# xUhEngwAng/I2V-Adapter-Unofficial

Hardware: AMD Instinct MI355X
Metric: denoising steps/sec @ 16fx512x512 SD1.5+I2V-Adapter (higher is better)
Workload: dtype f16

## Files before the change

### i2v-adapter-unofficial_amd/_lib.py

```python
import ctypes as C
import os

_HERE = os.path.dirname(os.path.abspath(__file__))
LIB_PATH = os.environ.get("I2V_LIB_PATH") or os.path.join(_HERE, "libi2v_hip.so")
ABI_VERSION = 27

I2V_EPI_NONE, I2V_EPI_GELU, I2V_EPI_GEGLU = 0, 1, 2
I2V_STORE_ROWMAJOR, I2V_STORE_ROWPERM, I2V_STORE_VT, I2V_STORE_VT_T = 0, 1, 2, 3
I2V_A_PLAIN, I2V_A_CONV3X3 = 0, 1
I2V_LORA_MAX_ADAPTERS, I2V_LORA_MAX_RANK = 8, 256
I2V_ROUTE_GENERIC, I2V_ROUTE_CONV_THIN, I2V_ROUTE_BIG_TILE, I2V_ROUTE_BIG_DEEP, I2V_ROUTE_BIG_SPLITK = 0, 1, 2, 3, 4
I2V_EXTRA_NONE, I2V_EXTRA_LNF, I2V_EXTRA_HILO, I2V_EXTRA_GNS, I2V_EXTRA_UPF = 0, 1, 2, 4, 8
I2V_TATTN_LDS_FORM, I2V_TATTN_REG_FORM = 0, 1
I2V_ADD_RES_MAX = 16
I2V_TAESD_PREP_IDENTITY, I2V_TAESD_PREP_UNIT, I2V_TAESD_PREP_CLAMP = 0, 1, 2


class HipLibraryError(RuntimeError):
    pass


class GemmParams(C.Structure):
    _fields_ = [
        ("a", C.c_void_p), ("lda", C.c_int64),
        ("a2", C.c_void_p), ("lda2", C.c_int64),
        ("k_split", C.c_int32), ("a_mode", C.c_int32),
        ("w", C.c_void_p), ("ldw", C.c_int64),
        ("bias", C.c_void_p),
        ("residual", C.c_void_p), ("ldr", C.c_int64),
        ("rowvec", C.c_void_p), ("ld_rowvec", C.c_int64), ("rows_per_vec", C.c_int32), ("rowvec_period", C.c_int32),
        ("ln_wsum", C.c_void_p), ("ln_eps", C.c_float),
        ("c", C.c_void_p), ("ldc", C.c_int64),
        ("M", C.c_int32), ("N", C.c_int32), ("K", C.c_int32),
        ("epilogue", C.c_int32), ("store_mode", C.c_int32),
        ("frames", C.c_int32), ("hw", C.c_int32),
        ("vt_len", C.c_int32), ("vt_ld", C.c_int32),
        ("out_scale", C.c_float),
        ("n_img", C.c_int32), ("in_h", C.c_int32), ("in_w", C.c_int32), ("cin", C.c_int32),
        ("out_h", C.c_int32), ("out_w", C.c_int32), ("stride", C.c_int32), ("upsample", C.c_int32),
        ("asym_pad", C.c_int32), ("conv_kblock", C.c_int32),
        ("w_batch_stride", C.c_int64), ("rows_per_w", C.c_int32),
        ("a_perm_frames", C.c_int32), ("a_perm_hw", C.c_int32),
        ("workspace", C.c_void_p), ("workspace_bytes", C.c_int64),
        ("c_is_f32", C.c_int32),
        ("gn_partial", C.c_void_p), ("gn_groups", C.c_int32),
        ("residual_lo", C.c_void_p), ("c_lo", C.c_void_p),
    ]


class GemmRoute(C.Structure):
    _fields_ = [
        ("family", C.c_int32), ("a_mode", C.c_int32),
        ("rows", C.c_int32), ("cols", C.c_int32), ("stages", C.c_int32),
        ("splits", C.c_int32), ("kps", C.c_int32),
        ("extra", C.c_int32), ("persistent", C.c_int32),
        ("generic_tile", C.c_int32), ("vec4", C.c_int32),
        ("epilogue", C.c_int32), ("store_mode", C.c_int32),
    ]

    def as_dict(self):
        return {name: int(getattr(self, name)) for name, _ in self._fields_}


class AttnParams(C.Structure):
    _fields_ = [
        ("q", C.c_void_p), ("q_row_stride", C.c_int64), ("q_batch_stride", C.c_int64),
        ("k", C.c_void_p), ("k_row_stride", C.c_int64), ("k_batch_stride", C.c_int64),
        ("vt", C.c_void_p), ("vt_row_stride", C.c_int64), ("vt_batch_stride", C.c_int64),
        ("o", C.c_void_p), ("o_row_stride", C.c_int64), ("o_batch_stride", C.c_int64),
        ("batch_q", C.c_int32), ("kv_group", C.c_int32), ("heads", C.c_int32), ("head_dim", C.c_int32),
        ("lq", C.c_int32), ("lk", C.c_int32),
        ("scale", C.c_float), ("accumulate", C.c_int32), ("acc_scale", C.c_float),
        ("lse", C.c_void_p),
    ]


class AttnBwdParams(C.Structure):
    _fields_ = [
        ("q", C.c_void_p), ("q_row_stride", C.c_int64), ("q_batch_stride", C.c_int64),
        ("qt", C.c_void_p), ("qt_row_stride", C.c_int64), ("qt_batch_stride", C.c_int64),
        ("k", C.c_void_p), ("k_row_stride", C.c_int64), ("k_batch_stride", C.c_int64),
        ("kt", C.c_void_p), ("kt_row_stride", C.c_int64), ("kt_batch_stride", C.c_int64),
        ("v", C.c_void_p), ("v_row_stride", C.c_int64), ("v_batch_stride", C.c_int64),
        ("dout", C.c_void_p), ("do_row_stride", C.c_int64), ("do_batch_stride", C.c_int64),
        ("doutt", C.c_void_p), ("dot_row_stride", C.c_int64), ("dot_batch_stride", C.c_int64),
        ("lse", C.c_void_p), ("delta", C.c_void_p),
        ("dq", C.c_void_p), ("dq_row_stride", C.c_int64), ("dq_batch_stride", C.c_int64),
        ("dk", C.c_void_p), ("dk_row_stride", C.c_int64), ("dk_batch_stride", C.c_int64),
        ("dv", C.c_void_p), ("dv_row_stride", C.c_int64), ("dv_batch_stride", C.c_int64),
        ("batch_q", C.c_int32), ("kv_group", C.c_int32), ("heads", C.c_int32), ("head_dim", C.c_int32),
        ("lq", C.c_int32), ("lk", C.c_int32),
        ("scale", C.c_float), ("kv_partitions", C.c_int32), ("dkv_partial", C.c_void_p),
    ]


class TAttnParams(C.Structure):
    _fields_ = [
        ("q", C.c_void_p), ("q_row_stride", C.c_int64),
        ("k", C.c_void_p), ("k_row_stride", C.c_int64),
        ("vt", C.c_void_p), ("vt_ld", C.c_int32),
        ("o", C.c_void_p), ("o_row_stride", C.c_int64),
        ("n_pixels", C.c_int32), ("frames", C.c_int32), ("heads", C.c_int32), ("head_dim", C.c_int32),
        ("scale", C.c_float),
    ]


class TAttnRoute(C.Structure):
    _fields_ = [
        ("form", C.c_int32), ("dqk", C.c_int32), ("dpv", C.c_int32),
        ("pf", C.c_int32), ("nqt", C.c_int32), ("blocks", C.c_int32),
    ]

    def as_dict(self):
        return {name: int(getattr(self, name)) for name, _ in self._fields_}


class MotionAttnParams(C.Structure):
    _fields_ = [
        ("x", C.c_void_p), ("ldx", C.c_int64),
        ("gamma", C.c_void_p),
        ("shift", C.c_void_p), ("ld_shift", C.c_int64),
        ("w_qkv", C.c_void_p),
        ("out", C.c_void_p), ("ldo", C.c_int64),
        ("rows", C.c_int64),
        ("channels", C.c_int32), ("heads", C.c_int32), ("head_dim", C.c_int32), ("frames", C.c_int32),
        ("eps", C.c_float), ("scale", C.c_float),
        ("w_o", C.c_void_p), ("b_o", C.c_void_p),
    ]


class CrossAttnFusedParams(C.Structure):
    _fields_ = [
        ("x", C.c_void_p), ("ldx", C.c_int64),
        ("gamma", C.c_void_p), ("beta", C.c_void_p),
        ("w_q", C.c_void_p),
        ("ctx_frag", C.c_void_p),
        ("out", C.c_void_p), ("ldo", C.c_int64),
        ("rows", C.c_int64), ("rows_per_ctx", C.c_int64),
        ("channels", C.c_int32), ("heads", C.c_int32), ("head_dim", C.c_int32), ("ctx_len", C.c_int32),
        ("eps", C.c_float), ("scale", C.c_float),
        ("ip_frag", C.c_void_p), ("ip_len", C.c_int32), ("ip_scale", C.c_float),
        ("w_o", C.c_void_p), ("b_o", C.c_void_p),
    ]


class FfFusedParams(C.Structure):
    _fields_ = [
        ("x", C.c_void_p), ("ldx", C.c_int64),
        ("gamma", C.c_void_p), ("beta", C.c_void_p),
        ("w1", C.c_void_p), ("b1", C.c_void_p),
        ("w2", C.c_void_p), ("b2", C.c_void_p),
        ("out", C.c_void_p), ("ldo", C.c_int64),
        ("rows", C.c_int64),
        ("channels", C.c_int32), ("inner", C.c_int32),
        ("eps", C.c_float),
        ("w3", C.c_void_p), ("b3", C.c_void_p),
        ("res2", C.c_void_p), ("ld_res2", C.c_int64),
        ("perm_frames", C.c_int32), ("perm_hw", C.c_int32),
        ("res2_lo", C.c_void_p), ("out_lo", C.c_void_p),
    ]


class LnQkvParams(C.Structure):
    _fields_ = [
        ("x", C.c_void_p), ("ldx", C.c_int64),
        ("gamma", C.c_void_p), ("beta", C.c_void_p),
        ("w", C.c_void_p),
        ("qk", C.c_void_p), ("ld_qk", C.c_int64),
        ("vt", C.c_void_p), ("vt_batch_stride", C.c_int64), ("vt_row_stride", C.c_int64),
        ("rows", C.c_int64), ("rows_per_image", C.c_int64),
        ("channels", C.c_int32), ("n_qk", C.c_int32),
        ("eps", C.c_float),
        ("x_image_stride", C.c_int64),
    ]


class UnetConfig(C.Structure):
    _fields_ = [
        ("in_channels", C.c_int32), ("out_channels", C.c_int32),
        ("block_out_channels", C.c_int32 * 4),
        ("layers_per_block", C.c_int32), ("num_attention_heads", C.c_int32),
        ("cross_attention_dim", C.c_int32), ("norm_num_groups", C.c_int32),
        ("motion_max_seq_length", C.c_int32), ("motion_num_attention_heads", C.c_int32),
        ("use_motion_mid_block", C.c_int32), ("ip_num_tokens", C.c_int32),
    ]


class UnetPlan(C.Structure):
    _fields_ = [
        ("batch", C.c_int32), ("frames", C.c_int32), ("height", C.c_int32), ("width", C.c_int32),
        ("ctx_len", C.c_int32), ("has_ip", C.c_int32),
    ]


class GnParams(C.Structure):
    _fields_ = [
        ("x", C.c_void_p), ("c1", C.c_int32),
        ("x2", C.c_void_p), ("c2", C.c_int32),
        ("gamma", C.c_void_p), ("beta", C.c_void_p),
        ("y", C.c_void_p),
        ("n_img", C.c_int32), ("hw", C.c_int32), ("groups", C.c_int32), ("frames_per_stat", C.c_int32),
        ("eps", C.c_float), ("silu", C.c_int32),
        ("out_perm", C.c_int32), ("frames", C.c_int32),
        ("workspace", C.c_void_p),
        ("gpartial_in", C.c_void_p), ("gpartial_rows", C.c_int32),
    ]


class LoraAdapter(C.Structure):
    _fields_ = [("down", C.c_void_p), ("up", C.c_void_p), ("rank", C.c_int32), ("scale", C.c_float)]


class LnParams(C.Structure):
    _fields_ = [
        ("x", C.c_void_p), ("ldx", C.c_int64),
        ("gamma", C.c_void_p), ("beta", C.c_void_p),
        ("pe", C.c_void_p), ("ld_pe", C.c_int64), ("pe_period", C.c_int32),
        ("y", C.c_void_p), ("ldy", C.c_int64),
        ("rows", C.c_int32), ("C", C.c_int32),
        ("eps", C.c_float),
        ("x_rows_per_batch", C.c_int32), ("x_batch_stride", C.c_int64),
    ]


class AddResidualsEntry(C.Structure):
    _fields_ = [("dst", C.c_void_p), ("dst_lo", C.c_void_p), ("skip", C.c_void_p), ("skip_lo", C.c_void_p), ("res", C.c_void_p),
                ("numel", C.c_int64)]


class AddResidualsParams(C.Structure):
    _fields_ = [("t", AddResidualsEntry * I2V_ADD_RES_MAX), ("n", C.c_int32), ("scale_rows", C.c_int32), ("scale_table", C.c_void_p),
                ("step_idx", C.c_void_p)]


class ConvC64Params(C.Structure):
    _fields_ = [
        ("x", C.c_void_p), ("ldx", C.c_int64),
        ("w", C.c_void_p), ("bias", C.c_void_p),
        ("residual", C.c_void_p), ("ldr", C.c_int64),
        ("out", C.c_void_p), ("ldo", C.c_int64),
        ("n_img", C.c_int32), ("height", C.c_int32), ("width", C.c_int32),
        ("cin", C.c_int32), ("cout", C.c_int32),
        ("relu_mid", C.c_int32), ("relu_out", C.c_int32),
        ("max_workgroups", C.c_int32),
    ]


_P = C.c_void_p
SIGNATURES = {
    "i2v_abi_version": (C.c_int, []),
    "i2v_last_error": (C.c_char_p, []),
    "i2v_gemm_f16": (C.c_int, [C.POINTER(GemmParams), _P]),
    "i2v_gemm_ln_supported": (C.c_int, [C.POINTER(GemmParams)]),
    "i2v_gemm_batch_supported": (C.c_int, [C.POINTER(GemmParams)]),
    "i2v_gemm_upconv_fold_supported": (C.c_int, [C.POINTER(GemmParams)]),
    "i2v_gemm_workspace_bytes": (C.c_int64, [C.POINTER(GemmParams)]),
    "i2v_gemm_gn_partial_rows": (C.c_int32, [C.POINTER(GemmParams)]),
    "i2v_gemm_route": (C.c_int, [C.POINTER(GemmParams), C.POINTER(GemmRoute)]),
    "i2v_gemm_last_route": (C.c_int, [C.POINTER(GemmRoute)]),
    "i2v_gemm_kernel_exists": (C.c_int, [C.POINTER(GemmRoute)]),
    "i2v_attention_f16": (C.c_int, [C.POINTER(AttnParams), _P]),
    "i2v_temporal_attention_f16": (C.c_int, [C.POINTER(TAttnParams), _P]),
    "i2v_temporal_attention_route": (C.c_int, [C.POINTER(TAttnParams), C.POINTER(TAttnRoute)]),
    "i2v_temporal_attention_last_route": (C.c_int, [C.POINTER(TAttnRoute)]),
    "i2v_tattn_kernel_exists": (C.c_int, [C.POINTER(TAttnRoute)]),
    "i2v_motion_attn_supported": (C.c_int32, [C.c_int64, C.c_int32, C.c_int32, C.c_int32, C.c_int32]),
    "i2v_motion_attn_pack_rows": (C.c_int32, [C.c_int32, C.c_int32]),
    "i2v_motion_attn_f16": (C.c_int, [C.POINTER(MotionAttnParams), _P]),
    "i2v_cross_attn_fused_supported": (C.c_int32, [C.c_int64, C.c_int32, C.c_int32, C.c_int32, C.c_int32, C.c_int64]),
    "i2v_cross_attn_fused_pack_rows": (C.c_int32, [C.c_int32, C.c_int32]),
    "i2v_cross_attn_fused_ctx_elems": (C.c_int64, [C.c_int32, C.c_int32, C.c_int32]),
    "i2v_cross_attn_fused_f16": (C.c_int, [C.POINTER(CrossAttnFusedParams), _P]),
    "i2v_ln_qkv_supported": (C.c_int32, [C.c_int64, C.c_int32, C.c_int32, C.c_int64]),
    "i2v_ln_qkv_f16": (C.c_int, [C.POINTER(LnQkvParams), _P]),
    "i2v_ff_fused_supported": (C.c_int32, [C.c_int64, C.c_int32, C.c_int32]),
    "i2v_ff_fused_tail_supported": (C.c_int32, [C.c_int64, C.c_int32, C.c_int32, C.c_int32, C.c_int32]),
    "i2v_ff_fused_f16": (C.c_int, [C.POINTER(FfFusedParams), _P]),
    "i2v_groupnorm_workspace_bytes": (C.c_int64, [C.c_int32, C.c_int32, C.c_int32]),
    "i2v_groupnorm_f16": (C.c_int, [C.POINTER(GnParams), _P]),
    "i2v_groupnorm_fold_f16": (C.c_int, [C.POINTER(GnParams), _P, C.c_int64, _P, C.c_int32, _P, _P, _P]),
    "i2v_layernorm_f16": (C.c_int, [C.POINTER(LnParams), _P]),
    "i2v_softmax_rows_f16": (C.c_int, [_P, C.c_int64, _P, C.c_int64, C.c_int32, C.c_int32, C.c_float, _P]),
    "i2v_nchw_to_tokens": (C.c_int, [_P, C.c_int32, _P, C.c_int32, C.c_int32, C.c_int32, C.c_int32, _P]),
    "i2v_tokens_to_nchw": (C.c_int, [_P, C.c_int32, C.c_int64, _P, C.c_int32, C.c_int32, C.c_int32, C.c_int32, _P]),
    "i2v_timestep_embedding": (C.c_int, [_P, _P, C.c_int32, _P, C.c_int32, C.c_int32, _P]),
    "i2v_silu_f16": (C.c_int, [_P, _P, C.c_int64, _P]),
    "i2v_repeat_rows_f16": (C.c_int, [_P, _P, C.c_int64, C.c_int64, C.c_int32, _P]),
    "i2v_copy3d_f16": (C.c_int, [_P, C.c_int64, C.c_int64, _P, C.c_int64, C.c_int64, C.c_int64, C.c_int64,
                                 C.c_int64, _P]),
    "i2v_pack_ctx_fragments_elems": (C.c_int64, [C.c_int32, C.c_int32, C.c_int32]),
    "i2v_pack_ctx_fragments_f16": (C.c_int, [_P, C.c_int64, _P, C.c_int64, C.c_int64, _P, C.c_int32, C.c_int32, C.c_int32, C.c_int32, _P]),
    "i2v_ddim_prep": (C.c_int, [_P, _P, _P, C.c_int32, C.c_int32, C.c_int32, C.c_int32, C.c_int32, C.c_int32, _P]),
    "i2v_gaussian_sample_f32": (C.c_int, [_P, _P, _P, C.c_int32, C.c_int32, C.c_int32, _P]),
    "i2v_first_frame_prior_f32": (C.c_int, [_P, _P, _P, _P, C.c_int32, C.c_int32, C.c_int32, C.c_int32, C.c_int32,
                                            C.c_float, C.c_float, C.c_float, C.c_float, C.c_float, _P]),
    "i2v_attention_lse_f32": (C.c_int, [C.POINTER(AttnParams), _P, _P]),
    "i2v_attention_bwd_f16": (C.c_int, [C.POINTER(AttnBwdParams), _P]),
    "i2v_transpose_f16": (C.c_int, [_P, C.c_int64, C.c_int64, _P, C.c_int64, C.c_int64, C.c_int32, C.c_int32, C.c_int32, _P]),
    "i2v_rowdot_heads_f32": (C.c_int, [_P, C.c_int64, _P, C.c_int64, _P, C.c_int64, C.c_int32, C.c_int32, C.c_int32, _P]),
    "i2v_layernorm_bwd_f16": (C.c_int, [_P, C.c_int64, _P, C.c_int64, _P, _P, C.c_int64, _P, C.c_int64, C.c_int32, C.c_int32,
                                        C.c_float, _P]),
    "i2v_geglu_bwd_f16": (C.c_int, [_P, C.c_int64, _P, C.c_int64, _P, C.c_int64, C.c_int64, C.c_int32, _P]),
    "i2v_geglu_f16": (C.c_int, [_P, C.c_int64, _P, C.c_int64, C.c_int64, C.c_int32, _P]),
    "i2v_colsum_f32": (C.c_int, [_P, C.c_int64, _P, C.c_int64, C.c_int32, _P]),
    "i2v_colsum_prod_f32": (C.c_int, [_P, C.c_int64, _P, C.c_int64, _P, C.c_int64, C.c_int32, _P]),
    "i2v_colsum_workspace_bytes": (C.c_int64, [C.c_int64, C.c_int32]),
    "i2v_colsum_det_f32": (C.c_int, [_P, C.c_int64, _P, C.c_int64, _P, C.c_int64, C.c_int32, _P, _P]),
    "i2v_masked_mse_grad_f16": (C.c_int, [_P, _P, _P, C.c_int64, C.c_int32, C.c_int32, C.c_int32, C.c_float, _P]),
    "i2v_masked_mse_grad_f32": (C.c_int, [_P, _P, _P, _P, C.c_int64, C.c_int32, C.c_int32, C.c_int32, C.c_float, _P]),
    "i2v_groupnorm_bwd_workspace_bytes": (C.c_int64, [C.c_int32, C.c_int32, C.c_int32]),
    "i2v_groupnorm_bwd_f16": (C.c_int, [C.POINTER(GnParams), _P, _P, _P, _P]),
    "i2v_add_f16": (C.c_int, [_P, _P, _P, C.c_int64, _P]),
    "i2v_permute_rows_f16": (C.c_int, [_P, _P, C.c_int64, C.c_int32, C.c_int32, C.c_int32, C.c_int32, _P]),
    "i2v_zero_insert2x_f16": (C.c_int, [_P, _P, C.c_int64, C.c_int32, C.c_int32, C.c_int32, _P]),
    "i2v_sum_pool2x_f16": (C.c_int, [_P, _P, C.c_int64, C.c_int32, C.c_int32, C.c_int32, _P]),
    "i2v_sumsq_f32": (C.c_int, [_P, C.c_int64, _P, _P]),
    "i2v_adamw_f32": (C.c_int, [_P, _P, _P, _P, C.c_int64, C.c_float, C.c_float, C.c_float, C.c_float, C.c_float, C.c_int32,
                                C.c_float, _P, C.c_float, _P]),
    "i2v_adamw_guarded_f32": (C.c_int, [_P, _P, _P, _P, C.c_int64, C.c_float, C.c_float, C.c_float, C.c_float, C.c_float,
                                        C.c_float, C.c_float, _P, C.c_int32, _P, _P, _P, _P]),
    "i2v_axpby_f32": (C.c_int, [_P, _P, C.c_float, C.c_float, C.c_int64, _P]),
    "i2v_select_row_f16": (C.c_int, [_P, C.c_int64, C.c_int32, _P, _P, C.c_int32, _P]),
    "i2v_ddim_cfg_step": (C.c_int, [_P, _P, C.c_int32, C.c_int64, _P, C.c_int32, _P, C.c_float, C.c_int32, C.c_int32,
                                    C.c_int32, C.c_int32, C.c_int32, _P]),
    "i2v_dpm_cfg_step": (C.c_int, [_P, _P, _P, C.c_int32, C.c_int64, _P, C.c_int32, _P, C.c_float, C.c_int32, C.c_int32,
                                   C.c_int32, C.c_int32, C.c_int32, _P]),
    "i2v_lcm_cfg_step": (C.c_int, [_P, _P, C.c_int32, _P, C.c_int32, C.c_int64, _P, C.c_int32, _P, C.c_float, C.c_int32, C.c_int32,
                                   C.c_int32, C.c_int32, C.c_int32, _P]),
    "i2v_freeu_f16": (C.c_int, [_P, _P, _P, _P, _P, _P, C.c_int32, C.c_int32, C.c_int32, C.c_int32, C.c_int32, C.c_float, C.c_float, _P]),
    "i2v_vae_tile_blend": (C.c_int, [_P, _P, _P, _P, C.c_int32, C.c_int32, C.c_int32, C.c_int32, C.c_int64, C.c_int32, C.c_int32, C.c_int32,
                                     C.c_int32, C.c_int32, _P, C.c_int32, C.c_int32, C.c_int32, C.c_int32, _P]),
    "i2v_lora_merge": (C.c_int, [_P, _P, C.c_int32, C.c_int32, C.c_int32, C.POINTER(LoraAdapter), C.c_int32, _P]),
    "i2v_freeinit_workspace_bytes": (C.c_int64, [C.c_int32, C.c_int32, C.c_int32, C.c_int32, C.c_int32]),
    "i2v_freeinit_mix": (C.c_int, [_P, _P, _P, _P, _P, _P, C.c_int64, C.c_int32, C.c_int32, C.c_int32, C.c_int32, C.c_int32, C.c_float,
                                   C.c_float, _P]),
    "i2v_freenoise_gather_f16": (C.c_int, [_P, C.c_int64, _P, C.c_int64, _P, C.c_int64, C.c_int32, C.c_int32, C.c_int32, C.c_int32, _P]),
    "i2v_freenoise_blend_f16": (C.c_int, [_P, C.c_int64, _P, C.c_int64, _P, _P, C.c_int64, C.c_int32, C.c_int32, C.c_int32, C.c_int32,
                                          C.c_int32, _P]),
    "i2v_clip_embed_f16": (C.c_int, [_P, _P, _P, _P, _P, C.c_int32, C.c_int32, C.c_int32, C.c_int32, C.c_int32, _P]),
    "i2v_clip_attention_f16": (C.c_int, [_P, C.c_int64, C.c_int32, C.c_int32, C.c_int32, _P, C.c_int64, C.c_int32, C.c_int32, C.c_int32,
                                         C.c_int32, C.c_float, _P]),
    "i2v_quick_gelu_f16": (C.c_int, [_P, _P, C.c_int64, _P]),
    "i2v_clip_patchify_f16": (C.c_int, [_P, _P, C.c_int64, C.c_int32, C.c_int32, C.c_int32, C.c_int32, _P]),
    "i2v_clip_vision_embed_f16": (C.c_int, [_P, _P, C.c_int64, _P, _P, C.c_int32, C.c_int32, C.c_int32, _P]),
    "i2v_clip_vision_attention_f16": (C.c_int, [_P, C.c_int64, C.c_int32, C.c_int32, C.c_int32, _P, C.c_int64, C.c_int32, C.c_int32,
                                                C.c_int32, C.c_int32, C.c_float, _P]),
    "i2v_perceiver_attention_f16": (C.c_int, [_P, C.c_int64, C.c_int32, _P, C.c_int64, C.c_int32, C.c_int32, C.c_int32, _P, C.c_int64,
                                              C.c_int32, C.c_int32, C.c_int32, _P, C.c_int64, C.c_int32, C.c_int32, C.c_int32, C.c_int32,
                                              C.c_float, _P]),
    "i2v_add_residuals_f16": (C.c_int, [C.POINTER(AddResidualsParams), _P]),
    "i2v_conv3x3_c64_f16": (C.c_int, [C.POINTER(ConvC64Params), _P]),
    "i2v_taesd_prep_f16": (C.c_int, [_P, C.c_int32, _P, C.c_int64, C.c_int32, C.c_int32, C.c_int32, C.c_int32, _P]),
    "i2v_pixel_unshuffle8_f16": (C.c_int, [_P, C.c_int32, _P, C.c_int32, C.c_int32, C.c_int32, C.c_int32, _P]),
    "i2v_avgpool2x_f16": (C.c_int, [_P, _P, C.c_int32, C.c_int32, C.c_int32, C.c_int32, _P]),
    "i2v_relu_f16": (C.c_int, [_P, _P, C.c_int64, _P]),
    "i2v_add_broadcast_residual_f16": (C.c_int, [_P, _P, _P, _P, _P, C.c_int64, C.c_int64, _P, C.c_int32, _P, _P]),
    "i2v_interp_rows_f16": (C.c_int, [_P, C.c_int64, C.c_int32, _P, _P, _P, _P, C.c_int64, C.c_int32, C.c_int32, _P]),
    "i2v_masked_renoise_f32": (C.c_int, [_P, _P, _P, _P, _P, C.c_int32, _P, C.c_int64, C.c_int32, C.c_int32, _P]),
    "i2v_weight_embeds_f16": (C.c_int, [_P, _P, _P, _P, C.c_int32, C.c_int32, C.c_int32, C.c_int64, C.c_int64, C.c_int32, _P]),
    "i2v_unet_create": (C.c_int, [C.POINTER(UnetConfig), C.POINTER(_P)]),
    "i2v_unet_destroy": (C.c_int, [_P]),
    "i2v_unet_set_weight": (C.c_int, [_P, C.c_char_p, _P, C.c_int32, C.c_int32, C.POINTER(C.c_int64)]),
    "i2v_unet_get_weight": (C.c_int, [_P, C.c_char_p, C.POINTER(_P), C.POINTER(C.c_int32), C.POINTER(C.c_int32),
                                      C.POINTER(C.c_int64)]),
    "i2v_unet_num_weights": (C.c_int64, [_P]),
    "i2v_unet_plan": (C.c_int, [_P, C.POINTER(UnetPlan)]),
    "i2v_unet_set_plan": (C.c_int, [_P, C.c_char_p, C.c_int64]),
    "i2v_unet_activation_bytes": (C.c_int64, [_P]),
    "i2v_unet_plan_launches": (C.c_int32, [_P]),
    "i2v_unet_plan_num_keys": (C.c_int32, [_P]),
    "i2v_unet_plan_key": (C.c_char_p, [_P, C.c_int32]),
    "i2v_unet_set_workspace": (C.c_int, [_P, _P, C.c_int64]),
    "i2v_unet_forward": (C.c_int, [_P, _P, _P, _P, _P, _P, _P]),
    "i2v_unet_abort_capture": (C.c_int, [_P]),
    "i2v_unet_run": (C.c_int, [_P, C.POINTER(_P), C.c_int32, _P]),
    "i2v_unet_capture_step": (C.c_int, [_P, _P]),
    "i2v_unet_end_capture": (C.c_int, [_P]),
    "i2v_unet_replay_step": (C.c_int, [_P, _P]),
    "i2v_unet_has_step": (C.c_int32, [_P]),
}

_lib = None


def load():
    global _lib
    if _lib is not None:
        return _lib
    if not os.path.exists(LIB_PATH):
        raise HipLibraryError(
            f"{LIB_PATH} not found: the HIP extension is not built.  Run `python __graft_entry__.py build` "
            "(needs hipcc, cross-compiles gfx950 without a GPU).  There is no CPU fallback for this path.")
    try:
        lib = C.CDLL(LIB_PATH)
    except OSError as e:
        raise HipLibraryError(f"cannot load {LIB_PATH}: {e}") from e
    for name, (res, args) in SIGNATURES.items():
        try:
            fn = getattr(lib, name)
        except AttributeError as e:
            raise HipLibraryError(f"{LIB_PATH} does not export `{name}` declared in include/i2v_hip.h") from e
        fn.restype = res
        fn.argtypes = args
    v = lib.i2v_abi_version()
    if v != ABI_VERSION:
        raise HipLibraryError(f"{LIB_PATH} has ABI version {v}, binding expects {ABI_VERSION}")
    _lib = lib
    return lib


def check(status: int, what: str):
    if status != 0:
        msg = load().i2v_last_error()
        raise HipLibraryError(f"{what} failed with status {status}: {msg.decode() if msg else ''}")
```

### i2v-adapter-unofficial_amd/blocks.py

```python
import math
import os
from typing import Optional

import torch
from torch import nn

from . import kernels as K
from . import streams
from ._lib import (I2V_EPI_GEGLU, I2V_EPI_GELU, I2V_EPI_NONE, I2V_STORE_ROWPERM, HipLibraryError)
from .checkpoint import PretrainedMixin

f16 = torch.float16


class HipModule(nn.Module):

    def __init__(self):
        super().__init__()
        self._packed = None
        self._packed_key = None

    def _pack(self):
        return {}

# ... 435 lines not shown
    def refresh_context_fragments(self, pc):
        hit = pc.frag.get(self)
        if hit is not None:
            k, vt, kip, vtip, lt, li = self.context_kv(pc, None)
            K.pack_ctx_fragments(k, vt, self.heads, lt, out=hit[0])
            if hit[1] is not None:
                K.pack_ctx_fragments(kip, vtip, self.heads, li, out=hit[1])

    def _cross(self, q, ctx_text, ctx_ip, batch_q, lq, kv_group, kv=None):
        k, vt, kip, vtip, lt, li = kv if kv is not None else self.context_kv(ctx_text, ctx_ip)
        o = K.attention(q, k, vt, batch_q=batch_q, lq=lq, lk=lt, heads=self.heads, head_dim=self.dim_head,
                        kv_group=kv_group, scale=self.scale)
        if kip is not None and self.ip_num_tokens:
            K.attention(q, kip, vtip, batch_q=batch_q, lq=lq, lk=li, heads=self.heads, head_dim=self.dim_head,
                        kv_group=kv_group, scale=self.scale, out=o, accumulate=True, acc_scale=self.ip_scale)
        return o

    def forward(self, hidden_states, encoder_hidden_states=None, attention_mask=None):
        if attention_mask is not None:
            raise NotImplementedError("attention masks are never passed on the hot path (SURVEY 8b)")
        p = self.packed()
        x = _as_f16_matrix(hidden_states)
        b, l, c = x.shape
        q = K.gemm(x.view(-1, c), p["wq"])
        ctx = x if encoder_hidden_states is None else _as_f16_matrix(encoder_hidden_states)
        ctx_ip = None
        if self.ip_num_tokens and encoder_hidden_states is not None:
            end = ctx.shape[1] - self.ip_num_tokens
            ctx_text = torch.empty((ctx.shape[0], end, ctx.shape[2]), dtype=f16, device=x.device)
            ctx_ip = torch.empty((ctx.shape[0], self.ip_num_tokens, ctx.shape[2]), dtype=f16, device=x.device)
            K.copy3d(ctx[:, :end], ctx_text)
            K.copy3d(ctx[:, end:], ctx_ip)
            ctx = ctx_text
        if b % ctx.shape[0] != 0:
            raise ValueError(f"context batch {ctx.shape[0]} does not divide query batch {b}")
        o = self._cross(q, ctx, ctx_ip, b, l, b // ctx.shape[0])
        out = K.gemm(o, p["wo"], p["bo"])
        return out.view(b, l, -1).to(hidden_states.dtype)


class GEGLU(nn.Module):
    def __init__(self, dim_in, dim_out, bias=True):
        super().__init__()
        self.proj = nn.Linear(dim_in, dim_out * 2, bias=bias)


class GELU(nn.Module):
    def __init__(self, dim_in, dim_out, approximate="none", bias=True):
        super().__init__()
        if approximate != "none":
            raise NotImplementedError("only erf GELU is implemented")
        self.proj = nn.Linear(dim_in, dim_out, bias=bias)


def ff_tail_operands(weight, bias, c_in, c_out):
    if c_in != c_out or not K.ff_fused_tail_supported(128, c_in, 4 * c_in):
        return None
    return K.pack_ff_tail(weight.detach().reshape(c_out, c_in), bias)


class FeedForward(HipModule):

    def __init__(self, dim, dim_out=None, mult=4, dropout=0.0, activation_fn="geglu", inner_dim=None, bias=True):
        super().__init__()
        if not bias:
            raise NotImplementedError("ff_bias=False is not on the hot path")
        inner_dim = int(dim * mult) if inner_dim is None else inner_dim
        dim_out = dim if dim_out is None else dim_out
        self.activation_fn = activation_fn
        if activation_fn == "geglu":
            act = GEGLU(dim, inner_dim, bias=bias)
        elif activation_fn == "gelu":
            act = GELU(dim, inner_dim, bias=bias)
        else:
            raise ValueError(f"unsupported activation_fn {activation_fn}")
        self.net = nn.ModuleList([act, nn.Dropout(dropout), nn.Linear(inner_dim, dim_out, bias=bias)])

    def _pack(self):
        proj = self.net[0].proj
        if self.activation_fn == "geglu":
            w1, b1 = pack_geglu(proj.weight.detach(), proj.bias.detach())
        else:
            w1, b1 = w16(proj.weight), w16(proj.bias)
        out = LazyPack(w1=w1, b1=b1, w2=w16(self.net[2].weight), b2=w16(self.net[2].bias))
        if self.activation_fn == "geglu" and K.ff_fused_supported(128, self.net[2].weight.shape[0], self.net[2].weight.shape[1]):
            out.lazy("fused", lambda proj=proj, lin=self.net[2]: K.pack_ff_fused(proj.weight, proj.bias, lin.weight, lin.bias))
        return out

    def _fwd(self, n2d, residual2d, **store):
        p = self.packed()
        epi = I2V_EPI_GEGLU if self.activation_fn == "geglu" else I2V_EPI_GELU
        h = K.gemm(n2d, p["w1"], p["b1"], epilogue=epi)
        return K.gemm(h, p["w2"], p["b2"], residual=residual2d, **store)

    def fused_supported(self, x2d):
        p = self.packed()
        return FUSED_FF and "fused" in p and K.ff_fused_supported(x2d.shape[0], x2d.shape[1], p["b1"].numel() // 2)

    def _fwd_fused(self, x2d, gamma32, beta32, eps, tail=None):
        return K.ff_fused(x2d, gamma32, beta32, self.packed()["fused"], eps=eps, tail=tail, precise=precise_stream())

    def tail_supported(self, x2d, tail):
        p = self.packed()
        return (FUSED_FF and FUSED_FF_TAIL and tail is not None and tail[0] is not None and "fused" in p and
                K.ff_fused_tail_supported(x2d.shape[0], x2d.shape[1], p["b1"].numel() // 2, tail[2], tail[3]))

    def fold_norm(self, norm):
        if self.activation_fn != "geglu":
            return None
        proj = self.net[0].proj
        return fold_layernorm_geglu(proj.weight, proj.bias, norm.weight, norm.bias)

    def _fwd_folded(self, x2d, eps, folded, **store):
        p = self.packed()
        wf, wsum, bf = folded
        h = K.gemm(x2d, wf, bf, epilogue=I2V_EPI_GEGLU, ln=(wsum, eps))
        return K.gemm(h, p["w2"], p["b2"], residual=x2d, **store)

    def folded_supported(self, x2d, eps, folded):
        wf, wsum, bf = folded
        return K.gemm(x2d, wf, bf, epilogue=I2V_EPI_GEGLU, ln=(wsum, eps), query_ln_support=True)

    def forward(self, hidden_states, scale: float = 1.0):
        x = _as_f16_matrix(hidden_states)
        shp = x.shape
        return self._fwd(x.view(-1, shp[-1]), None).view(*shp[:-1], -1).to(hidden_states.dtype)


class SinusoidalPositionalEmbedding(nn.Module):

    def __init__(self, embed_dim: int, max_seq_length: int = 32):
        super().__init__()
        self.embed_dim, self.max_seq_length = embed_dim, max_seq_length
        self.register_buffer("pe", self._table(embed_dim, max_seq_length))

    @staticmethod
    def _table(embed_dim, max_seq_length):
        position = torch.arange(max_seq_length, device="cpu").unsqueeze(1)
        div_term = torch.exp(torch.arange(0, embed_dim, 2, device="cpu") * (-math.log(10000.0) / embed_dim))
        pe = torch.zeros(1, max_seq_length, embed_dim, device="cpu")
        pe[0, :, 0::2] = torch.sin(position * div_term)
        pe[0, :, 1::2] = torch.cos(position * div_term)
        return pe

    def reset_table_(self):
        with torch.no_grad():
            self.pe.copy_(self._table(self.embed_dim, self.max_seq_length).to(self.pe.dtype))


FUSED_MOTION_ATTN = os.environ.get("I2V_MOTION_FUSED", "1") != "0"
FUSED_FF = os.environ.get("I2V_FF_FUSED", "1") != "0"
FUSED_FF_TAIL = os.environ.get("I2V_FF_TAIL", "1") != "0"
FUSED_ATTN_OUT = os.environ.get("I2V_ATTN_OUTP", "1") != "0"


class TemporalTransformerBlock(HipModule):

    def __init__(self, dim, num_attention_heads, attention_head_dim, dropout=0.0, cross_attention_dim=None,
                 activation_fn="geglu", attention_bias=False, double_self_attention=True,
                 norm_elementwise_affine=True, norm_eps=1e-5, positional_embeddings="sinusoidal",
                 num_positional_embeddings=32, **_unused):
        super().__init__()
        if cross_attention_dim is not None or not double_self_attention or positional_embeddings != "sinusoidal":
            raise NotImplementedError("motion modules use double self-attention with sinusoidal positions (A9)")
        self.dim, self.heads, self.dim_head = dim, num_attention_heads, attention_head_dim
        self.eps = norm_eps
        self.max_len = num_positional_embeddings
        self.pos_embed = SinusoidalPositionalEmbedding(dim, max_seq_length=num_positional_embeddings)
        self.norm1 = nn.LayerNorm(dim, elementwise_affine=norm_elementwise_affine, eps=norm_eps)
        self.attn1 = Attention(query_dim=dim, heads=num_attention_heads, dim_head=attention_head_dim,
                               dropout=dropout, bias=attention_bias)
        self.norm2 = nn.LayerNorm(dim, elementwise_affine=norm_elementwise_affine, eps=norm_eps)
        self.attn2 = Attention(query_dim=dim, heads=num_attention_heads, dim_head=attention_head_dim,
                               dropout=dropout, bias=attention_bias)
        self.norm3 = nn.LayerNorm(dim, elementwise_affine=norm_elementwise_affine, eps=norm_eps)
        self.ff = FeedForward(dim, dropout=dropout, activation_fn=activation_fn)
        self._plan = LnFoldPlan()
        self.free_noise = None

    def _pack(self):
        p = LazyPack(pe=w16(self.pos_embed.pe[0]))
        for i, (norm, attn) in enumerate(((self.norm1, self.attn1), (self.norm2, self.attn2)), 1):
            p[f"g{i}"], p[f"b{i}"] = w16(norm.weight), w16(norm.bias)
            p[f"wqk{i}"] = w16(torch.cat([attn.to_q.weight, attn.to_k.weight], dim=0))
            p[f"wv{i}"] = w16(attn.to_v.weight)
            p[f"wo{i}"], p[f"bo{i}"] = w16(attn.to_out[0].weight), w16(attn.to_out[0].bias)
        p["g3"], p["b3"] = w16(self.norm3.weight), w16(self.norm3.bias)
        pe = self.pos_embed.pe[0].detach().float()
        for i, (norm, attn) in enumerate(((self.norm1, self.attn1), (self.norm2, self.attn2)), 1):
            wqk = torch.cat([attn.to_q.weight, attn.to_k.weight], dim=0)
            p[f"f_wqk{i}"], p[f"f_sqk{i}"], p[f"f_cqk{i}"] = fold_layernorm(wqk, None, norm.weight, norm.bias)
            p[f"f_peqk{i}"] = (pe @ wqk.detach().float().T).to(f16).contiguous()
            p[f"f_wv{i}"], p[f"f_sv{i}"], p[f"f_cv{i}"] = fold_layernorm(attn.to_v.weight, None, norm.weight, norm.bias)
            p[f"f_pev{i}"] = (pe @ attn.to_v.weight.detach().float().T).T.to(f16).contiguous()
        p["f_ff"] = self.ff.fold_norm(self.norm3)
        for i, attn in enumerate((self.attn1, self.attn2), 1):
            p.lazy(f"wqkv{i}", lambda attn=attn, heads=self.heads: K.pack_motion_qkv(attn.to_q.weight, attn.to_k.weight, attn.to_v.weight, heads))
            p.lazy(f"wo_frag{i}", lambda attn=attn, heads=self.heads: K.pack_attn_out(attn.to_out[0].weight, attn.to_out[0].bias, heads))
        self._ma_tables = {}
        p.lazy("g3_f32", lambda n3=self.norm3: n3.weight.detach().float().contiguous())
        p.lazy("b3_f32", lambda n3=self.norm3: n3.bias.detach().float().contiguous())
        return p

    def _fold_ok(self, t, frames, sites=("attn", "ff")):
        def probe_attn():
            p = self.packed()
            if frames & (frames - 1):
                return False
            return (K.gemm(t, p["f_wqk1"], p["f_cqk1"], ln=(p["f_sqk1"], self.eps), rowvec=p["f_peqk1"],
                           rowvec_period=frames, query_ln_support=True) and
                    K.project_vt(t, p["f_wv1"], frames, bias=p["f_cv1"], ln=(p["f_sv1"], self.eps), pe_t=p["f_pev1"],
                                 pe_period=frames, query_ln_support=True))

        def probe_ff():
            p = self.packed()
            return p["f_ff"] is not None and self.ff.folded_supported(t, self.eps, p["f_ff"])

        key = (t.shape[0], frames)
        return (self._plan.get(("attn",) + key, probe_attn) if "attn" in sites else False,
                self._plan.get(("ff",) + key, probe_ff) if "ff" in sites else False)

    def _fwd(self, t, n_pixels, frames, tail=None):
        fn = self.free_noise
        if fn is not None and frames > fn.context_length:
            return self._fwd_windows(t, n_pixels, frames, fn, tail)
        if frames > self.max_len:
            raise ValueError(f"num_frames {frames} exceeds the positional table ({self.max_len})")
        fold_attn, fold_ff = self._fold_ok(t, frames)
        return self._fwd_ff(self._fwd_attn(t, n_pixels, frames, fold_attn), fold_ff, tail)

    def _fwd_windows(self, t, n_pixels, frames, fn, tail):
        from . import free_noise
        length = fn.context_length
        starts, idx, coef = free_noise.tables(frames, fn, t.device)
        windows = starts.numel()
        tw = K.freenoise_gather(t, starts, n_pixels=n_pixels, frames=frames, length=length)
        tw = self._fwd_attn(tw, n_pixels * windows, length, self._fold_ok(tw, length, sites=("attn",))[0])
        t = K.freenoise_blend(tw, idx, coef, n_pixels=n_pixels, windows=windows, length=length)
        return self._fwd_ff(t, self._fold_ok(t, frames, sites=("ff",))[1], tail)

    def _fwd_attn(self, t, n_pixels, frames, fold_attn):
        p = self.packed()
        c = self.dim
        overlap = t.shape[0] <= streams.MAX_ROWS
        fused = FUSED_MOTION_ATTN and K.motion_attn_supported(t.shape[0], c, self.heads, self.dim_head, frames)
        for i in (1, 2):
            if fused:
                tab = self._ma_tables.get((i, frames))
                if tab is None:
                    tab = self._ma_tables[(i, frames)] = K.motion_attn_tables(p[f"g{i}"], p[f"b{i}"], p["pe"], frames)
                if FUSED_ATTN_OUT:
                    t = K.motion_attn(t, tab[0], tab[1], p[f"wqkv{i}"], heads=self.heads, head_dim=self.dim_head, frames=frames,
                                      eps=self.eps, out_proj=p[f"wo_frag{i}"])
                    continue
                o = K.motion_attn(t, tab[0], tab[1], p[f"wqkv{i}"], heads=self.heads, head_dim=self.dim_head, frames=frames,
                                  eps=self.eps)
                t = K.gemm(o, p[f"wo{i}"], p[f"bo{i}"], residual=t)
                continue
            n = None if fold_attn else K.layernorm(t, p[f"g{i}"], p[f"b{i}"], self.eps, pe=p["pe"], pe_period=frames)
            with streams.fork(overlap, t.device) as fk:
                with fk.side():
                    if fold_attn:
                        vt = K.project_vt(t, p[f"f_wv{i}"], frames, bias=p[f"f_cv{i}"], ln=(p[f"f_sv{i}"], self.eps),
                                          pe_t=p[f"f_pev{i}"], pe_period=frames)
                    else:
                        vt = K.project_vt(n, p[f"wv{i}"], frames)
                if fold_attn:
                    qk = K.gemm(t, p[f"f_wqk{i}"], p[f"f_cqk{i}"], ln=(p[f"f_sqk{i}"], self.eps),
                                rowvec=p[f"f_peqk{i}"], rowvec_period=frames)
                else:
                    qk = K.gemm(n, p[f"wqk{i}"])
            o = K.temporal_attention(qk[:, :c], qk[:, c:], vt, n_pixels=n_pixels, frames=frames, heads=self.heads,
                                     head_dim=self.dim_head, scale=self.dim_head ** -0.5)
            t = K.gemm(o, p[f"wo{i}"], p[f"bo{i}"], residual=t)
        return t

    def _fwd_ff(self, t, fold_ff, tail):
        p = self.packed()

        def ret(v, applied=False):
            return v if tail is None else (v, applied)
        if self.ff.fused_supported(t):
            if self.ff.tail_supported(t, tail):
                return ret(self.ff._fwd_fused(t, p["g3_f32"], p["b3_f32"], self.eps, tail=tail), True)
            return ret(self.ff._fwd_fused(t, p["g3_f32"], p["b3_f32"], self.eps))
        if fold_ff:
            return ret(self.ff._fwd_folded(t, self.eps, p["f_ff"]))
        n = K.layernorm(t, p["g3"], p["b3"], self.eps)
        return ret(self.ff._fwd(n, t))


class TransformerTemporalModel(HipModule):

    def __init__(self, num_attention_heads=16, attention_head_dim=88, in_channels=None, out_channels=None,
                 num_layers=1, dropout=0.0, norm_num_groups=32, cross_attention_dim=None, attention_bias=False,
                 activation_fn="geglu", norm_elementwise_affine=True, double_self_attention=True,
                 positional_embeddings=None, num_positional_embeddings=None):
        super().__init__()
        inner_dim = num_attention_heads * attention_head_dim
        self.in_channels, self.inner_dim = in_channels, inner_dim
        self.groups = norm_num_groups
        self.norm = nn.GroupNorm(norm_num_groups, in_channels, eps=1e-6, affine=True)
        self.proj_in = nn.Linear(in_channels, inner_dim)
        self.transformer_blocks = nn.ModuleList([
            TemporalTransformerBlock(inner_dim, num_attention_heads, attention_head_dim, dropout=dropout,
                                     cross_attention_dim=cross_attention_dim, activation_fn=activation_fn,
                                     attention_bias=attention_bias, double_self_attention=double_self_attention,
                                     norm_elementwise_affine=norm_elementwise_affine,
                                     positional_embeddings=positional_embeddings,
                                     num_positional_embeddings=num_positional_embeddings)
            for _ in range(num_layers)])
        self.proj_out = nn.Linear(inner_dim, in_channels)

    def _pack(self):
        p = LazyPack(g=w16(self.norm.weight), b=w16(self.norm.bias), wi=w16(self.proj_in.weight),
                     bi=w16(self.proj_in.bias), wo=w16(self.proj_out.weight), bo=w16(self.proj_out.bias))
        p.lazy("tail", lambda po=self.proj_out, ci=self.inner_dim, co=self.in_channels: ff_tail_operands(po.weight, po.bias, ci, co))
        return p

    def set_free_noise(self, settings):
        for blk in self.transformer_blocks:
            if settings is not None and settings.context_length > blk.max_len:
                raise ValueError(f"`context_length` {settings.context_length} exceeds the motion module's num_positional_embeddings "
                                 f"({blk.max_len})")
        for blk in self.transformer_blocks:
            blk.free_noise = settings

    def _fwd(self, x, num_frames):
        p = self.packed()
        n, hh, ww, c = x.shape
        if n % num_frames != 0:
            raise ValueError(f"batch {n} is not a multiple of num_frames {num_frames}")
        n_pixels = (n // num_frames) * hh * ww
        t = gn_proj_in(x, p["g"], p["b"], self.groups, 1e-6, p["wi"], p["bi"], frames=num_frames)
        applied = False
        for j, blk in enumerate(self.transformer_blocks):
            if j + 1 == len(self.transformer_blocks):
                t, applied = blk._fwd(t, n_pixels, num_frames, tail=(p["tail"], K.sview(x, -1, c), num_frames, hh * ww))
            else:
                t = blk._fwd(t, n_pixels, num_frames)
        if applied:
            return K.sview(t, n, hh, ww, c)
        out = K.gemm(t, p["wo"], p["bo"], residual=K.sview(x, -1, c), store=I2V_STORE_ROWPERM, frames=num_frames,
                     hw=hh * ww, precise=precise_stream())
        return K.sview(out, n, hh, ww, c)

    def forward(self, hidden_states, encoder_hidden_states=None, num_frames: int = 1, return_dict=False, **_unused):
        return (from_tokens(self._fwd(to_tokens(hidden_states), num_frames), hidden_states.dtype),)


class ImageProjection(HipModule):

    def __init__(self, image_embed_dim=768, cross_attention_dim=768, num_image_text_embeds=4):
        super().__init__()
        self.num_image_text_embeds = num_image_text_embeds
        self.cross_attention_dim = cross_attention_dim
        self.image_embeds = nn.Linear(image_embed_dim, num_image_text_embeds * cross_attention_dim)
        self.norm = nn.LayerNorm(cross_attention_dim)

    def _pack(self):
        return dict(w=w16(self.image_embeds.weight), b=w16(self.image_embeds.bias), g=w16(self.norm.weight),
                    be=w16(self.norm.bias))

    def forward(self, image_embeds):
        p = self.packed()
        x = _as_f16_matrix(image_embeds)
        y = K.gemm(x, p["w"], p["b"]).view(-1, self.cross_attention_dim)
        y = K.layernorm(y, p["g"], p["be"], self.norm.eps)
        return y.view(x.shape[0], self.num_image_text_embeds, self.cross_attention_dim)


class _ResamplerAttention(nn.Module):

    def __init__(self, dim, inner):
        super().__init__()
        self.to_q, self.to_k, self.to_v = (nn.Linear(dim, inner, bias=False) for _ in range(3))
        self.to_out = nn.ModuleList([nn.Linear(inner, dim, bias=False), nn.Dropout(0.0)])


class _ResamplerFeedForward(nn.Module):

    def __init__(self, dim, inner):
        super().__init__()
        self.net = nn.ModuleList([GELU(dim, inner, bias=False), nn.Dropout(0.0), nn.Linear(inner, dim, bias=False)])


class Resampler(HipModule):

    DIM_HEAD, MAX_QUERIES, MAX_KEYS = 64, 64, 288

    def __init__(self, embed_dims=768, output_dims=1024, hidden_dims=1280, depth=4, dim_head=64, heads=16, num_queries=8, ffn_ratio=4):
        super().__init__()
        if dim_head != self.DIM_HEAD:
            raise NotImplementedError(f"dim_head {dim_head}: the attention kernel (i2v_perceiver_attention_f16) implements head_dim "
                                      f"{self.DIM_HEAD} only")
        if not 1 <= num_queries <= self.MAX_QUERIES:
            raise NotImplementedError(f"num_queries {num_queries}: the attention kernel (i2v_perceiver_attention_f16) takes 1 to "
                                      f"{self.MAX_QUERIES} queries")
        inner_ff = int(hidden_dims * ffn_ratio)
        if embed_dims % 8 or output_dims % 8 or hidden_dims % 8 or inner_ff % 8 or inner_ff != hidden_dims * ffn_ratio:
            raise NotImplementedError(f"embed_dims {embed_dims}, output_dims {output_dims}, hidden_dims {hidden_dims} and hidden_dims * "
                                      f"ffn_ratio {hidden_dims * ffn_ratio} must be multiples of 8 (i2v_gemm_f16)")
        self.embed_dims, self.output_dims, self.hidden_dims = embed_dims, output_dims, hidden_dims
# ... 514 lines not shown
```

### i2v-adapter-unofficial_amd/csrc/handle.hip

```cpp
#include <string.h>

#include <map>
#include <string>
#include <vector>

#include "common.h"

namespace {

constexpr uint32_t PLAN_MAGIC = 0x50563249u;
constexpr uint32_t PLAN_VERSION = 1;
struct PlanHeader {
  uint32_t magic, version, abi, n_ops, n_keys, n_relocs;
  int32_t batch, frames, height, width, ctx_len, has_ip;
  uint64_t arena_bytes;
  uint32_t io_read_mask, reserved;
  uint64_t keys_off, ops_off, relocs_off, payload_off, payload_bytes, total_bytes;
};
struct PlanOp {
  uint32_t entry, payload_off, payload_bytes, reloc_begin, reloc_count, struct_bytes;
};
struct PlanReloc {
  uint32_t offset, kind, index, pad;
  uint64_t addend;
};
enum { RELOC_ARENA = 0, RELOC_WEIGHT = 1, RELOC_IO = 2 };

enum Entry {
  E_GEMM = 0, E_ATTN, E_TATTN, E_MOTION_ATTN, E_CROSS_ATTN_FUSED, E_LN_QKV, E_FF_FUSED, E_GROUPNORM, E_LAYERNORM,
  E_GROUPNORM_FOLD, E_NCHW_TO_TOKENS, E_TOKENS_TO_NCHW, E_TIMESTEP_EMBEDDING, E_SILU, E_REPEAT_ROWS, E_COPY3D, E_SELECT_ROW,
  E_PACK_CTX_FRAGMENTS, E_DDIM_PREP, E_DDIM_CFG_STEP, E_DPM_CFG_STEP, E_FREEU, E_LCM_CFG_STEP, E_FREENOISE_GATHER,
  E_FREENOISE_BLEND, E_COUNT
};
struct EntryInfo {
  const char* name;
  uint32_t struct_bytes;
  uint32_t slots;
};
const EntryInfo ENTRIES[E_COUNT] = {
    {"i2v_gemm_f16", sizeof(i2v_gemm_params), 0},
    {"i2v_attention_f16", sizeof(i2v_attn_params), 0},
    {"i2v_temporal_attention_f16", sizeof(i2v_tattn_params), 0},
    {"i2v_motion_attn_f16", sizeof(i2v_motion_attn_params), 0},
    {"i2v_cross_attn_fused_f16", sizeof(i2v_cross_attn_fused_params), 0},
    {"i2v_ln_qkv_f16", sizeof(i2v_ln_qkv_params), 0},
    {"i2v_ff_fused_f16", sizeof(i2v_ff_fused_params), 0},
    {"i2v_groupnorm_f16", sizeof(i2v_gn_params), 0},
    {"i2v_layernorm_f16", sizeof(i2v_ln_params), 0},
    {"i2v_groupnorm_fold_f16", sizeof(i2v_gn_params), 6},
    {"i2v_nchw_to_tokens", 0, 7},
    {"i2v_tokens_to_nchw", 0, 8},
    {"i2v_timestep_embedding", 0, 6},
    {"i2v_silu_f16", 0, 3},
    {"i2v_repeat_rows_f16", 0, 5},
    {"i2v_copy3d_f16", 0, 9},
    {"i2v_select_row_f16", 0, 6},
    {"i2v_pack_ctx_fragments_f16", 0, 10},
    {"i2v_ddim_prep", 0, 9},
    {"i2v_ddim_cfg_step", 0, 13},
    {"i2v_dpm_cfg_step", 0, 14},
    {"i2v_freeu_f16", 0, 13},
    {"i2v_lcm_cfg_step", 0, 15},
    {"i2v_freenoise_gather_f16", 0, 10},
    {"i2v_freenoise_blend_f16", 0, 12},
};
inline uint32_t pad8(uint32_t n) { return (n + 7u) & ~7u; }

}

struct i2v_unet {
  i2v_unet_config cfg;
  struct weight { const void* ptr; int32_t dtype, ndim; int64_t shape[4]; };
  std::map<std::string, weight> weights;
  uint64_t weights_generation = 0;
  i2v_unet_plan_t plan;
  bool planned = false;
  std::vector<unsigned char> blob;
  std::vector<std::string> keys;
  std::vector<const void*> key_ptr;
  uint64_t bound_generation = ~0ull;
  void* arena = nullptr;
  int64_t arena_bytes = 0;
  hipStream_t capture_stream = nullptr;
  bool capturing = false;
  hipGraph_t graph = nullptr;
  hipGraphExec_t exec = nullptr;

  const PlanHeader* header() const { return blob.empty() ? nullptr : reinterpret_cast<const PlanHeader*>(blob.data()); }
};

namespace {
void drop_step(i2v_unet* h) {
  if (h->exec) (void)hipGraphExecDestroy(h->exec);
  if (h->graph) (void)hipGraphDestroy(h->graph);
  h->exec = nullptr;
  h->graph = nullptr;
}
void drop_plan(i2v_unet* h) {
  h->blob.clear();
  h->keys.clear();
  h->key_ptr.clear();
  h->bound_generation = ~0ull;
}
}

extern "C" int i2v_unet_create(const i2v_unet_config* cfg, i2v_unet** out) {
  I2V_CHECK_ARG(cfg != nullptr && out != nullptr, "i2v_unet_create: null argument");
  I2V_CHECK_ARG(cfg->in_channels > 0 && cfg->out_channels > 0 && cfg->layers_per_block > 0 && cfg->num_attention_heads > 0 &&
                    cfg->cross_attention_dim > 0 && cfg->norm_num_groups > 0 && cfg->motion_max_seq_length > 0 &&
                    cfg->motion_num_attention_heads > 0 && cfg->ip_num_tokens >= 0,
                "i2v_unet_create: non-positive size in the configuration");
  for (int i = 0; i < 4; ++i) {
    const int c = cfg->block_out_channels[i];
    I2V_CHECK_ARG(c > 0 && c % cfg->norm_num_groups == 0 && c % cfg->num_attention_heads == 0 && c % 8 == 0,
                  "i2v_unet_create: block_out_channels[%d] = %d must be a positive multiple of 8, of norm_num_groups (%d) and of "
                  "num_attention_heads (%d)", i, c, cfg->norm_num_groups, cfg->num_attention_heads);
  }
  i2v_unet* h = new (std::nothrow) i2v_unet();
  if (h == nullptr) I2V_FAIL(I2V_ERR_UNSUPPORTED, "i2v_unet_create: out of host memory");
  h->cfg = *cfg;
  *out = h;
  return I2V_OK;
}

extern "C" int i2v_unet_abort_capture(i2v_unet* h) {
  I2V_CHECK_ARG(h != nullptr, "i2v_unet_abort_capture: null handle");
  if (!h->capturing) return I2V_OK;
  h->capturing = false;
  hipGraph_t g = nullptr;
  (void)hipStreamEndCapture(h->capture_stream, &g);
  (void)hipGetLastError();
  if (g) (void)hipGraphDestroy(g);
  return I2V_OK;
}

extern "C" int i2v_unet_destroy(i2v_unet* h) {
  if (h == nullptr) return I2V_OK;
  (void)i2v_unet_abort_capture(h);
  drop_step(h);
  delete h;
  return I2V_OK;
}

extern "C" int i2v_unet_set_weight(i2v_unet* h, const char* key, const void* ptr, int32_t dtype, int32_t ndim, const int64_t* shape) {
  I2V_CHECK_ARG(h != nullptr && key != nullptr && key[0] != 0 && ptr != nullptr, "i2v_unet_set_weight: null handle, key or pointer");
  I2V_CHECK_ARG(dtype == I2V_DTYPE_F16 || dtype == I2V_DTYPE_F32, "i2v_unet_set_weight: dtype %d of `%s` (fp16 = 0 or fp32 = 1)", dtype, key);
  I2V_CHECK_ARG(ndim >= 0 && ndim <= 4 && (ndim == 0 || shape != nullptr), "i2v_unet_set_weight: ndim %d of `%s`", ndim, key);
  i2v_unet::weight w = {ptr, dtype, ndim, {1, 1, 1, 1}};
  for (int i = 0; i < ndim; ++i) {
    I2V_CHECK_ARG(shape[i] > 0, "i2v_unet_set_weight: shape[%d] = %lld of `%s`", i, (long long)shape[i], key);
    w.shape[i] = shape[i];
  }
  I2V_CHECK_ARG((reinterpret_cast<uintptr_t>(ptr) & (dtype == I2V_DTYPE_F16 ? 1 : 3)) == 0, "i2v_unet_set_weight: `%s` is misaligned", key);
  try {
    h->weights[std::string(key)] = w;
  } catch (...) {
    I2V_FAIL(I2V_ERR_UNSUPPORTED, "i2v_unet_set_weight: out of host memory registering `%s`", key);
  }
  ++h->weights_generation;
  return I2V_OK;
}

extern "C" int i2v_unet_get_weight(const i2v_unet* h, const char* key, const void** ptr, int32_t* dtype, int32_t* ndim, int64_t* shape) {
  I2V_CHECK_ARG(h != nullptr && key != nullptr && ptr != nullptr, "i2v_unet_get_weight: null argument");
  std::map<std::string, i2v_unet::weight>::const_iterator it;
  try {
    it = h->weights.find(std::string(key));
  } catch (...) {
    I2V_FAIL(I2V_ERR_UNSUPPORTED, "i2v_unet_get_weight: out of host memory looking up `%s`", key);
  }
  if (it == h->weights.end()) {
    *ptr = nullptr;
    return I2V_OK;
  }
  *ptr = it->second.ptr;
  if (dtype) *dtype = it->second.dtype;
  if (ndim) *ndim = it->second.ndim;
  if (shape)
    for (int i = 0; i < it->second.ndim; ++i) shape[i] = it->second.shape[i];
  return I2V_OK;
}

extern "C" int64_t i2v_unet_num_weights(const i2v_unet* h) { return h ? (int64_t)h->weights.size() : 0; }

extern "C" int i2v_unet_plan(i2v_unet* h, const i2v_unet_plan_t* plan) {
  I2V_CHECK_ARG(h != nullptr && plan != nullptr, "i2v_unet_plan: null argument");
  I2V_CHECK_ARG(!h->capturing, "i2v_unet_plan: a capture is in progress (i2v_unet_end_capture / i2v_unet_abort_capture first)");
  I2V_CHECK_ARG(plan->batch > 0 && plan->frames > 0 && plan->height > 0 && plan->width > 0 && plan->ctx_len > 0,
                "i2v_unet_plan: non-positive size");
  I2V_CHECK_ARG(plan->frames <= h->cfg.motion_max_seq_length, "i2v_unet_plan: num_frames %d exceeds the positional table (%d)",
                plan->frames, h->cfg.motion_max_seq_length);
  I2V_CHECK_ARG(!plan->has_ip || h->cfg.ip_num_tokens > 0, "i2v_unet_plan: has_ip without image tokens in the configuration");
  drop_step(h);
  if (!h->planned || memcmp(&h->plan, plan, sizeof(*plan)) != 0) drop_plan(h);
  h->plan = *plan;
  h->planned = true;
  return I2V_OK;
}

extern "C" int i2v_unet_set_plan(i2v_unet* h, const void* blob, int64_t bytes) {
  I2V_CHECK_ARG(h != nullptr && blob != nullptr, "i2v_unet_set_plan: null argument");
  I2V_CHECK_ARG(h->planned, "i2v_unet_set_plan: i2v_unet_plan (the problem the plan was recorded for) first");
  I2V_CHECK_ARG(!h->capturing, "i2v_unet_set_plan: a capture is in progress");
  I2V_CHECK_ARG(bytes >= (int64_t)sizeof(PlanHeader), "i2v_unet_set_plan: %lld bytes is not a launch plan", (long long)bytes);
  PlanHeader hd;
  memcpy(&hd, blob, sizeof(hd));
  I2V_CHECK_ARG(hd.magic == PLAN_MAGIC && hd.version == PLAN_VERSION, "i2v_unet_set_plan: bad magic / version (%#x, %u)", hd.magic, hd.version);
  I2V_CHECK_ARG(hd.abi == I2V_ABI_VERSION, "i2v_unet_set_plan: the plan was recorded against ABI %u, this library is ABI %d", hd.abi, I2V_ABI_VERSION);
  I2V_CHECK_ARG(hd.total_bytes == (uint64_t)bytes, "i2v_unet_set_plan: the blob says %llu bytes, %lld were passed", (unsigned long long)hd.total_bytes,
                (long long)bytes);
  I2V_CHECK_ARG(hd.batch == h->plan.batch && hd.frames == h->plan.frames && hd.height == h->plan.height && hd.width == h->plan.width &&
                    hd.ctx_len == h->plan.ctx_len && hd.has_ip == h->plan.has_ip,
                "i2v_unet_set_plan: recorded for (batch %d, frames %d, %d x %d, ctx %d, ip %d), planned (%d, %d, %d x %d, %d, %d)", hd.batch,
                hd.frames, hd.height, hd.width, hd.ctx_len, hd.has_ip, h->plan.batch, h->plan.frames, h->plan.height, h->plan.width,
                h->plan.ctx_len, h->plan.has_ip);
  const uint64_t total = hd.total_bytes;
  auto inside = [&](uint64_t off, uint64_t len) { return off % 8 == 0 && off <= total && len <= total - off; };
// ... 41 lines not shown
    drop_plan(h);
    h->blob.assign(base, base + total);
    h->keys.swap(keys);
    h->key_ptr.assign(h->keys.size(), nullptr);
  } catch (...) {
    drop_plan(h);
    I2V_FAIL(I2V_ERR_UNSUPPORTED, "i2v_unet_set_plan: out of host memory");
  }
  return I2V_OK;
}

extern "C" int64_t i2v_unet_activation_bytes(const i2v_unet* h) {
  const PlanHeader* hd = h ? h->header() : nullptr;
  return hd ? (int64_t)hd->arena_bytes : 0;
}
extern "C" int32_t i2v_unet_plan_launches(const i2v_unet* h) {
  const PlanHeader* hd = h ? h->header() : nullptr;
  return hd ? (int32_t)hd->n_ops : 0;
}
extern "C" int32_t i2v_unet_plan_num_keys(const i2v_unet* h) { return h ? (int32_t)h->keys.size() : 0; }
extern "C" const char* i2v_unet_plan_key(const i2v_unet* h, int32_t i) {
  return (h && i >= 0 && i < (int32_t)h->keys.size()) ? h->keys[(size_t)i].c_str() : nullptr;
}

extern "C" int i2v_unet_set_workspace(i2v_unet* h, void* arena, int64_t bytes) {
  I2V_CHECK_ARG(h != nullptr, "i2v_unet_set_workspace: null handle");
  I2V_CHECK_ARG(!h->capturing, "i2v_unet_set_workspace: a capture is in progress");
  I2V_CHECK_ARG((arena == nullptr) == (bytes == 0) && bytes >= 0 && (reinterpret_cast<uintptr_t>(arena) & 255) == 0,
                "i2v_unet_set_workspace: the arena must be 256-byte aligned with a positive size (or NULL, 0)");
  drop_step(h);
  h->arena = arena;
  h->arena_bytes = bytes;
  return I2V_OK;
}

extern "C" int i2v_unet_run(i2v_unet* h, const void* const* io_args, int32_t n_io, i2v_stream_t stream);

extern "C" int i2v_unet_forward(i2v_unet* h, const void* sample, const void* timesteps, const void* context, const void* image_embeds,
                                void* out, i2v_stream_t stream) {
  const void* io[I2V_IO_SLOTS] = {sample, timesteps, context, image_embeds, out};
  return i2v_unet_run(h, io, I2V_IO_SLOTS, stream);
}

extern "C" int i2v_unet_run(i2v_unet* h, const void* const* io_args, int32_t n_io, i2v_stream_t stream) {
  I2V_CHECK_ARG(h != nullptr && (n_io == 0 || io_args != nullptr) && n_io >= 0 && n_io <= I2V_IO_SLOTS, "i2v_unet_forward: null handle / argument array");
  const PlanHeader* hd = h->header();
  I2V_CHECK_ARG(hd != nullptr, "i2v_unet_forward: no launch plan (i2v_unet_set_plan)");
  I2V_CHECK_ARG(hd->arena_bytes == 0 || (h->arena != nullptr && (uint64_t)h->arena_bytes >= hd->arena_bytes),
                "i2v_unet_forward: the arena holds %lld bytes, the plan needs %llu (i2v_unet_set_workspace)", (long long)h->arena_bytes,
                (unsigned long long)hd->arena_bytes);
  const void* io[I2V_IO_SLOTS] = {nullptr, nullptr, nullptr, nullptr, nullptr};
  for (int s = 0; s < n_io; ++s) io[s] = io_args[s];
  static const char* io_name[I2V_IO_SLOTS] = {"sample", "timesteps", "context", "image_embeds", "out"};
  for (int s = 0; s < I2V_IO_SLOTS; ++s)
    I2V_CHECK_ARG(!((hd->io_read_mask >> s) & 1u) || io[s] != nullptr, "i2v_unet_forward: `%s` (argument %d) is NULL and the plan uses it",
                  io_name[s], s);
  if (h->bound_generation != h->weights_generation) {
    for (size_t i = 0; i < h->keys.size(); ++i) {
      const auto it = h->weights.find(h->keys[i]);
      if (it == h->weights.end()) {
        h->bound_generation = ~0ull;
        I2V_FAIL(I2V_ERR_INVALID_ARG, "i2v_unet_forward: weight `%s` of the launch plan is not registered (i2v_unet_set_weight)", h->keys[i].c_str());
      }
      h->key_ptr[i] = it->second.ptr;
    }
    h->bound_generation = h->weights_generation;
  }
  const unsigned char* base = h->blob.data();
  const PlanOp* ops = reinterpret_cast<const PlanOp*>(base + hd->ops_off);
  const PlanReloc* rel = reinterpret_cast<const PlanReloc*>(base + hd->relocs_off);
  const unsigned char* payload = base + hd->payload_off;
  alignas(16) unsigned char buf[1024];
  for (uint32_t i = 0; i < hd->n_ops; ++i) {
    const PlanOp& op = ops[i];
    if (op.payload_bytes > sizeof(buf)) I2V_FAIL(I2V_ERR_UNSUPPORTED, "i2v_unet_forward: launch %u has a %u-byte parameter block", i, op.payload_bytes);
    memcpy(buf, payload + op.payload_off, op.payload_bytes);
    for (uint32_t r = op.reloc_begin; r < op.reloc_begin + op.reloc_count; ++r) {
      const PlanReloc& q = rel[r];
      const unsigned char* target = q.kind == RELOC_ARENA    ? reinterpret_cast<const unsigned char*>(h->arena)
                                    : q.kind == RELOC_WEIGHT ? reinterpret_cast<const unsigned char*>(h->key_ptr[q.index])
                                                             : reinterpret_cast<const unsigned char*>(io[q.index]);
      if (target == nullptr) I2V_FAIL(I2V_ERR_INVALID_ARG, "i2v_unet_forward: launch %u reads `%s`, which is NULL", i, io_name[q.index]);
      const uint64_t v = reinterpret_cast<uint64_t>(target) + q.addend;
      memcpy(buf + q.offset, &v, 8);
    }
    const unsigned char* sl = buf + pad8(op.struct_bytes);
    auto P = [&](int k) { void* v; memcpy(&v, sl + 8 * k, 8); return v; };
    auto I = [&](int k) { int64_t v; memcpy(&v, sl + 8 * k, 8); return v; };
    auto F = [&](int k) { double v; memcpy(&v, sl + 8 * k, 8); return (float)v; };
    int rc = I2V_OK;
    switch (op.entry) {
      case E_GEMM: rc = i2v_gemm_f16(reinterpret_cast<const i2v_gemm_params*>(buf), stream); break;
      case E_ATTN: rc = i2v_attention_f16(reinterpret_cast<const i2v_attn_params*>(buf), stream); break;
      case E_TATTN: rc = i2v_temporal_attention_f16(reinterpret_cast<const i2v_tattn_params*>(buf), stream); break;
      case E_MOTION_ATTN: rc = i2v_motion_attn_f16(reinterpret_cast<const i2v_motion_attn_params*>(buf), stream); break;
      case E_CROSS_ATTN_FUSED: rc = i2v_cross_attn_fused_f16(reinterpret_cast<const i2v_cross_attn_fused_params*>(buf), stream); break;
      case E_LN_QKV: rc = i2v_ln_qkv_f16(reinterpret_cast<const i2v_ln_qkv_params*>(buf), stream); break;
      case E_FF_FUSED: rc = i2v_ff_fused_f16(reinterpret_cast<const i2v_ff_fused_params*>(buf), stream); break;
      case E_GROUPNORM: rc = i2v_groupnorm_f16(reinterpret_cast<const i2v_gn_params*>(buf), stream); break;
      case E_LAYERNORM: rc = i2v_layernorm_f16(reinterpret_cast<const i2v_ln_params*>(buf), stream); break;
      case E_GROUPNORM_FOLD:
        rc = i2v_groupnorm_fold_f16(reinterpret_cast<const i2v_gn_params*>(buf), P(0), I(1), P(2), (int32_t)I(3), P(4), P(5), stream);
        break;
      case E_NCHW_TO_TOKENS:
        rc = i2v_nchw_to_tokens(P(0), (int32_t)I(1), P(2), (int32_t)I(3), (int32_t)I(4), (int32_t)I(5), (int32_t)I(6), stream);
        break;
      case E_TOKENS_TO_NCHW:
        rc = i2v_tokens_to_nchw(P(0), (int32_t)I(1), I(2), P(3), (int32_t)I(4), (int32_t)I(5), (int32_t)I(6), (int32_t)I(7), stream);
        break;
      case E_TIMESTEP_EMBEDDING:
        rc = i2v_timestep_embedding(reinterpret_cast<const float*>(P(0)), reinterpret_cast<const int32_t*>(P(1)), (int32_t)I(2), P(3),
                                    (int32_t)I(4), (int32_t)I(5), stream);
        break;
      case E_SILU: rc = i2v_silu_f16(P(0), P(1), I(2), stream); break;
      case E_REPEAT_ROWS: rc = i2v_repeat_rows_f16(P(0), P(1), I(2), I(3), (int32_t)I(4), stream); break;
      case E_COPY3D: rc = i2v_copy3d_f16(P(0), I(1), I(2), P(3), I(4), I(5), I(6), I(7), I(8), stream); break;
      case E_SELECT_ROW:
        rc = i2v_select_row_f16(P(0), I(1), (int32_t)I(2), reinterpret_cast<const int32_t*>(P(3)), P(4), (int32_t)I(5), stream);
        break;
      case E_PACK_CTX_FRAGMENTS:
        rc = i2v_pack_ctx_fragments_f16(P(0), I(1), P(2), I(3), I(4), P(5), (int32_t)I(6), (int32_t)I(7), (int32_t)I(8), (int32_t)I(9), stream);
        break;
      case E_DDIM_PREP:
        rc = i2v_ddim_prep(reinterpret_cast<float*>(P(0)), reinterpret_cast<const float*>(P(1)), P(2), (int32_t)I(3), (int32_t)I(4), (int32_t)I(5),
                           (int32_t)I(6), (int32_t)I(7), (int32_t)I(8), stream);
        break;
      case E_DDIM_CFG_STEP:
        rc = i2v_ddim_cfg_step(reinterpret_cast<float*>(P(0)), P(1), (int32_t)I(2), I(3), reinterpret_cast<const float*>(P(4)), (int32_t)I(5),
                               reinterpret_cast<int32_t*>(P(6)), F(7), (int32_t)I(8), (int32_t)I(9), (int32_t)I(10), (int32_t)I(11), (int32_t)I(12),
                               stream);
        break;
      case E_DPM_CFG_STEP:
        rc = i2v_dpm_cfg_step(reinterpret_cast<float*>(P(0)), reinterpret_cast<float*>(P(1)), P(2), (int32_t)I(3), I(4),
                              reinterpret_cast<const float*>(P(5)), (int32_t)I(6), reinterpret_cast<int32_t*>(P(7)), F(8), (int32_t)I(9),
                              (int32_t)I(10), (int32_t)I(11), (int32_t)I(12), (int32_t)I(13), stream);
        break;
      case E_FREEU:
        rc = i2v_freeu_f16(P(0), P(1), P(2), P(3), P(4), P(5), (int32_t)I(6), (int32_t)I(7), (int32_t)I(8), (int32_t)I(9), (int32_t)I(10), F(11),
                           F(12), stream);
        break;
      case E_LCM_CFG_STEP:
        rc = i2v_lcm_cfg_step(reinterpret_cast<float*>(P(0)), reinterpret_cast<const float*>(P(1)), (int32_t)I(2), P(3), (int32_t)I(4), I(5),
                              reinterpret_cast<const float*>(P(6)), (int32_t)I(7), reinterpret_cast<int32_t*>(P(8)), F(9), (int32_t)I(10),
                              (int32_t)I(11), (int32_t)I(12), (int32_t)I(13), (int32_t)I(14), stream);
        break;
      case E_FREENOISE_GATHER:
        rc = i2v_freenoise_gather_f16(P(0), I(1), P(2), I(3), reinterpret_cast<const int32_t*>(P(4)), I(5), (int32_t)I(6), (int32_t)I(7),
                                      (int32_t)I(8), (int32_t)I(9), stream);
        break;
      case E_FREENOISE_BLEND:
        rc = i2v_freenoise_blend_f16(P(0), I(1), P(2), I(3), reinterpret_cast<const int32_t*>(P(4)), reinterpret_cast<const float*>(P(5)), I(6),
                                     (int32_t)I(7), (int32_t)I(8), (int32_t)I(9), (int32_t)I(10), (int32_t)I(11), stream);
        break;
      default: I2V_FAIL(I2V_ERR_UNSUPPORTED, "i2v_unet_forward: launch %u names entry point %u", i, op.entry);
    }
    if (rc != I2V_OK) return rc;
  }
  return I2V_OK;
}

extern "C" int i2v_unet_capture_step(i2v_unet* h, i2v_stream_t stream) {
  I2V_CHECK_ARG(h != nullptr && stream != nullptr, "i2v_unet_capture_step: null handle or the null stream (capture needs a stream of its own)");
  I2V_CHECK_ARG(h->planned, "i2v_unet_capture_step: i2v_unet_plan first");
  I2V_CHECK_ARG(!h->capturing, "i2v_unet_capture_step: a capture is already in progress (i2v_unet_abort_capture discards it)");
  drop_step(h);
  hipStream_t s = reinterpret_cast<hipStream_t>(stream);
  const hipError_t e = hipStreamBeginCapture(s, hipStreamCaptureModeRelaxed);
  if (e != hipSuccess) {
    (void)hipGetLastError();
    I2V_FAIL(I2V_ERR_LAUNCH, "i2v_unet_capture_step: hipStreamBeginCapture: %s", hipGetErrorString(e));
  }
  h->capture_stream = s;
  h->capturing = true;
  return I2V_OK;
}

extern "C" int i2v_unet_end_capture(i2v_unet* h) {
  I2V_CHECK_ARG(h != nullptr && h->capturing, "i2v_unet_end_capture: no capture in progress");
  h->capturing = false;
  hipError_t e = hipStreamEndCapture(h->capture_stream, &h->graph);
  if (e != hipSuccess || h->graph == nullptr) {
    (void)hipGetLastError();
    h->graph = nullptr;
    I2V_FAIL(I2V_ERR_LAUNCH, "i2v_unet_end_capture: hipStreamEndCapture: %s", hipGetErrorString(e));
  }
  e = hipGraphInstantiate(&h->exec, h->graph, nullptr, nullptr, 0);
  if (e != hipSuccess) {
    (void)hipGetLastError();
    drop_step(h);
    I2V_FAIL(I2V_ERR_LAUNCH, "i2v_unet_end_capture: hipGraphInstantiate: %s", hipGetErrorString(e));
  }
  return I2V_OK;
}

extern "C" int i2v_unet_replay_step(i2v_unet* h, i2v_stream_t stream) {
  I2V_CHECK_ARG(h != nullptr && h->exec != nullptr, "i2v_unet_replay_step: no captured step");
  const hipError_t e = hipGraphLaunch(h->exec, reinterpret_cast<hipStream_t>(stream));
  if (e != hipSuccess) {
    (void)hipGetLastError();
    I2V_FAIL(I2V_ERR_LAUNCH, "i2v_unet_replay_step: hipGraphLaunch: %s", hipGetErrorString(e));
  }
  return I2V_OK;
}

extern "C" int32_t i2v_unet_has_step(const i2v_unet* h) { return h != nullptr && h->exec != nullptr; }
```

### i2v-adapter-unofficial_amd/csrc/motion_attn.hip

```cpp
#include <stdlib.h>

#include <type_traits>

#include "common.h"

namespace {

__device__ __forceinline__ f32x4 mfma16x16x16(f16x4 a, f16x4 b, f32x4 c) {
  return __builtin_amdgcn_mfma_f32_16x16x16f16(a, b, c, 0, 0, 0);
}

__device__ __forceinline__ void ma_dma16(__amdgpu_buffer_rsrc_t rsrc, f16* lds_wave_base, unsigned voff, unsigned soff) {
  __builtin_amdgcn_raw_ptr_buffer_load_lds(rsrc, (__attribute__((address_space(3))) void*)lds_wave_base, 16, voff, soff, 0, 0);
}
__device__ __forceinline__ int ma_opaque(int v) {
  asm volatile("" : "+v"(v));
  return v;
}

constexpr int MA_PIX = 8;
constexpr int MA_F = 16;
constexpr int MA_PD = 3;
constexpr int MA_AD = 4;

struct ma_args {
  const void* x; int64_t ldx;
  const void* gamma; const void* shift; int64_t ld_shift;
  const void* w;
  void* out; int64_t ldo;
  float eps;
  const void* ctx_frag;
  int32_t lt; int32_t tiles_per_ctx;
  const void* ip_frag; int32_t ip_len; float ip_scale;
  const void* w_o; const void* b_o;
};

constexpr int MA_KT = 5;

template <int C, int D, int H, bool CROSS, int F = 16, bool OUTP = false>
__global__ __launch_bounds__(64 * H) void motion_attn_kernel(const ma_args p, const float scale_log2, const int ntiles,
                                                             long long* __restrict__ stamps) {
  constexpr int DT = (D + 15) / 16, DP = 16 * DT, KS = C / 32, NJ = C / 64, PARTS = CROSS ? 1 : 3;
  static_assert(C % 64 == 0 && H == 8, "one wave per head, 8 lanes x C / 64 chunks per row in the LayerNorm pass");
  static_assert(F == 8 || F == 16 || F == 32, "frames per pixel");
  extern __shared__ __attribute__((aligned(16))) f16 panels[];
  const int tid = threadIdx.x, lane = tid & 63, wave = __builtin_amdgcn_readfirstlane(tid >> 6);
  const int g = lane >> 4, l15 = lane & 15, sub = lane & 7;
  const f16* __restrict__ X = reinterpret_cast<const f16*>(p.x);
  const float* __restrict__ gamma = reinterpret_cast<const float*>(p.gamma);
  const float* __restrict__ shift = reinterpret_cast<const float*>(p.shift);
#ifdef I2V_MA_STAMPS
  long long stamp[8];
#define MA_STAMP(k) stamp[k] = __builtin_amdgcn_s_memtime()
#else
#define MA_STAMP(k)
#endif

  auto fetch_rows = [&](const int tile, f16* panel) {
    const f16* base = X + ((int64_t)tile * (MA_PIX * MA_F) + 16 * wave) * p.ldx;
    const auto rs = __builtin_amdgcn_make_buffer_rsrc(const_cast<f16*>(base), 0, (int)((15 * p.ldx + C) * 2), 0x00020000);
    const int ln = ma_opaque(lane);
    const unsigned voff = (unsigned)(((ln >> 3) * p.ldx + (ln & 7) * 8) * 2);
#pragma unroll
    for (int half = 0; half < 2; ++half)
#pragma unroll
      for (int j = 0; j < NJ; ++j)
        ma_dma16(rs, panel + 16 * wave * C + (half * NJ + j) * 512, voff, (unsigned)((8 * half * p.ldx + 8 * j * 8) * 2));
  };
  auto normalise_rows = [&](f16* panel) {
    f16x8 xv[2][NJ];
#pragma unroll
    for (int half = 0; half < 2; ++half)
#pragma unroll
      for (int j = 0; j < NJ; ++j) xv[half][j] = *reinterpret_cast<const f16x8*>(panel + 16 * wave * C + ((half * NJ + j) * 64 + lane) * 8);
    const float* gp = gamma;
    const float* sp = shift;
    asm volatile("" : "+s"(gp), "+s"(sp));
    f32x4 ga[NJ][2];
#pragma unroll
    for (int j = 0; j < NJ; ++j) {
      ga[j][0] = *reinterpret_cast<const f32x4*>(gp + (sub + 8 * j) * 8);
      ga[j][1] = *reinterpret_cast<const f32x4*>(gp + (sub + 8 * j) * 8 + 4);
    }
#pragma unroll
    for (int half = 0; half < 2; ++half) {
      const int row = 16 * wave + 8 * half + (lane >> 3);
      const float* sh = sp + (int64_t)((16 * wave + 8 * half + (lane >> 3)) & (F - 1)) * p.ld_shift;
      f32x4 sv[NJ][2];
#pragma unroll
      for (int j = 0; j < NJ; ++j) {
        sv[j][0] = *reinterpret_cast<const f32x4*>(sh + (sub + 8 * j) * 8);
        sv[j][1] = *reinterpret_cast<const f32x4*>(sh + (sub + 8 * j) * 8 + 4);
      }
      float v[NJ][8];
      float s = 0.f;
#pragma unroll
      for (int j = 0; j < NJ; ++j)
#pragma unroll
        for (int e = 0; e < 8; ++e) {
          v[j][e] = (float)xv[half][j][e];
          s += v[j][e];
        }
      s = sum_lanes8(s);
      const float mean = s / (float)C;
      float q = 0.f;
#pragma unroll
      for (int j = 0; j < NJ; ++j)
#pragma unroll
        for (int e = 0; e < 8; ++e) {
          v[j][e] -= mean;
          q = fmaf(v[j][e], v[j][e], q);
        }
      q = sum_lanes8(q);
      const float rstd = rsqrtf(q / (float)C + p.eps);
#pragma unroll
      for (int j = 0; j < NJ; ++j) {
        const int ch = sub + 8 * j;
        f16x8 o;
#pragma unroll
        for (int e = 0; e < 8; ++e) o[e] = (f16)fmaf(v[j][e] * rstd, ga[j][e >> 2][e & 3], sv[j][e >> 2][e & 3]);
        *reinterpret_cast<f16x8*>(panel + row * C + ((ch ^ (row & 7)) * 8)) = o;
      }
    }
  };

  const auto rs_w = __builtin_amdgcn_make_buffer_rsrc(const_cast<void*>(p.w), 0, H * PARTS * DP * C * 2, 0x00020000);
  const int w_lane = lane * 16, w_wave = wave * (PARTS * DP * C * 2);
  const int sw = l15 & 7;
  const int swz[2] = {(g ^ sw) * 8, ((4 + g) ^ sw) * 8};
  f32x4 acc[MA_PIX][DT];
  auto zero_init = [](const int, const int) { return f32x4{0.f, 0.f, 0.f, 0.f}; };
  auto no_hook = []() {};
  auto project = [&](const f16* panel, const __amdgpu_buffer_rsrc_t rs, const int wp, auto transposed, auto init, auto hook) {
    constexpr bool TR = decltype(transposed)::value;
    auto ldw = [&](const int s, const int t) {
      return __builtin_bit_cast(f16x8, __builtin_amdgcn_raw_buffer_load_b128(rs, w_lane, wp + (s * DT + t) * 1024, 0));
    };
    const f16* alane = panel + l15 * C;
    f16x8 wf[MA_PD][DT];
#pragma unroll
    for (int pix = 0; pix < MA_PIX; ++pix)
#pragma unroll
      for (int t = 0; t < DT; ++t) acc[pix][t] = init(pix, t);
#pragma unroll
    for (int s = 0; s < MA_PD - 1; ++s)
#pragma unroll
      for (int t = 0; t < DT; ++t) wf[s][t] = ldw(s, t);
    __builtin_amdgcn_sched_barrier(0);
    constexpr int AD = MA_AD, NI = KS * MA_PIX;
    auto lda = [&](const int i) {
      return *reinterpret_cast<const f16x8*>(alane + 16 * (i % MA_PIX) * C + 64 * ((i / MA_PIX) >> 1) + swz[(i / MA_PIX) & 1]);
    };
    f16x8 af[AD + 1];
#pragma unroll
    for (int i = 0; i < AD; ++i) af[i] = lda(i);
#pragma unroll
    for (int i = 0; i < NI; ++i) {
      const int s = i / MA_PIX, pix = i % MA_PIX;
      if (pix == 0 && s + MA_PD - 1 < KS) {
#pragma unroll
        for (int t = 0; t < DT; ++t) wf[(s + MA_PD - 1) % MA_PD][t] = ldw(s + MA_PD - 1, t);
      }
#ifndef I2V_MA_HOOK_S
#define I2V_MA_HOOK_S 0
#endif
      if (pix == 0 && s == I2V_MA_HOOK_S) hook();
      if (i + AD < NI) af[(i + AD) % (AD + 1)] = lda(i + AD);
#pragma unroll
      for (int t = 0; t < DT; ++t)
        acc[pix][t] = TR ? mfma16x16x32(wf[s % MA_PD][t], af[i % (AD + 1)], acc[pix][t])
                         : mfma16x16x32(af[i % (AD + 1)], wf[s % MA_PD][t], acc[pix][t]);
      __builtin_amdgcn_sched_barrier(0);
    }
  };
  auto to_half = [](const f32x4 a) { return f16x4{(f16)a[0], (f16)a[1], (f16)a[2], (f16)a[3]}; };
  static_assert(DT == 3 && D == 40, "store pattern of three 16-channel tiles holding 40 channels");
  auto store_tiles = [&](f16* orow, const int g, const u32x2 (&oh)[DT]) {
    u32x2 a = oh[0], b = oh[1], c2 = oh[2], d2 = oh[2];
    asm volatile("s_nop 1\n\tv_permlane16_swap_b32 %0, %1\n\tv_permlane16_swap_b32 %2, %3\n\t"
                 "v_permlane16_swap_b32 %4, %5\n\tv_permlane16_swap_b32 %6, %7"
                 : "+v"(a[0]), "+v"(b[0]), "+v"(a[1]), "+v"(b[1]), "+v"(c2[0]), "+v"(d2[0]), "+v"(c2[1]), "+v"(d2[1]));
    const u32x4 v01 = {a[0], a[1], b[0], b[1]};
    const u32x4 v2 = {c2[0], c2[1], d2[0], d2[1]};
#ifdef I2V_MA_NOSTORE
    if (p.ldo < 0)
#endif
    {
      *reinterpret_cast<u32x4*>(orow + ((g & 1) ? 16 + 4 * (g - 1) : 4 * g)) = v01;
      if (g == 0) *reinterpret_cast<u32x4*>(orow + 32) = v2;
    }
  };

  static_assert(D % 8 == 0, "a head's channels are whole 16-byte chunks of a panel row");
  auto stash_o = [&](f16* pw, const int pix, const u32x2 (&oh)[DT]) {
    const int ln = ma_opaque(lane), g2 = ln >> 4, r15 = ln & 15;
    f16* dst = pw + (16 * pix + r15) * C + 4 * (g2 & 1);
#pragma unroll
    for (int t = 0; t < DT; ++t)
      if (16 * t + 4 * g2 < D) *reinterpret_cast<u32x2*>(dst + (((wave * (D / 8) + 2 * t + (g2 >> 1)) ^ (r15 & 7)) * 8)) = oh[t];
  };
  auto out_project = [&](const f16* pr, const int tile) {
    const auto rs_o = __builtin_amdgcn_make_buffer_rsrc(const_cast<void*>(p.w_o), 0, H * DP * C * 2, 0x00020000);
    const auto rs_b = __builtin_amdgcn_make_buffer_rsrc(const_cast<void*>(p.b_o), 0, C * 4, 0x00020000);
    const f16* base = X + (int64_t)tile * (MA_PIX * MA_F) * p.ldx;
    const auto rs_x = __builtin_amdgcn_make_buffer_rsrc(const_cast<f16*>(base), 0, (int)(((MA_PIX * MA_F - 1) * p.ldx + C) * 2), 0x00020000);
    const int ln = ma_opaque(lane), sg = ln >> 4, sl15 = ln & 15;
    f32x4 bo[DT];
#pragma unroll
    for (int t = 0; t < DT; ++t)
      bo[t] = __builtin_bit_cast(f32x4, __builtin_amdgcn_raw_buffer_load_b128(
                                            rs_b, 16 * t + 4 * sg < D ? (unsigned)((wave * D + 16 * t + 4 * sg) * 4) : 0x80000000u, 0, 0));
    u32x2 res[MA_PIX][DT];
    project(pr, rs_o, wave * (DP * C * 2), std::true_type{}, [&](const int, const int t) { return bo[t]; }, [&]() {
#pragma unroll
      for (int pix = 0; pix < MA_PIX; ++pix)
#pragma unroll
        for (int t = 0; t < DT; ++t) {
#ifdef I2V_MA_NORES
          res[pix][t] = u32x2{0u, 0u};
#else
          const unsigned voff = 16 * t + 4 * sg < D ? (unsigned)((((16 * pix + sl15) * p.ldx) + wave * D + 16 * t + 4 * sg) * 2) : 0x80000000u;
          res[pix][t] = __builtin_bit_cast(u32x2, __builtin_amdgcn_raw_buffer_load_b64(rs_x, voff, 0, 0));
#endif
        }
    });
    f16* __restrict__ O = reinterpret_cast<f16*>(p.out) + (int64_t)tile * (MA_PIX * MA_F) * p.ldo + wave * D;
#pragma unroll
    for (int pix = 0; pix < MA_PIX; ++pix) {
      u32x2 oh[DT];
#pragma unroll
      for (int t = 0; t < DT; ++t) {
        const f16x4 r = __builtin_bit_cast(f16x4, res[pix][t]);
        const f32x4 v = {acc[pix][t][0] + (float)r[0], acc[pix][t][1] + (float)r[1], acc[pix][t][2] + (float)r[2], acc[pix][t][3] + (float)r[3]};
        oh[t] = __builtin_bit_cast(u32x2, to_half(v));
      }
      store_tiles(O + (int64_t)(16 * pix + sl15) * p.ldo, sg, oh);
    }
  };

  int tile = blockIdx.x;
  if (tile >= ntiles) return;
  MA_STAMP(0);
  fetch_rows(tile, panels);
  asm volatile("s_waitcnt vmcnt(0)" ::: "memory");
  normalise_rows(panels);
  MA_STAMP(1);
  lds_barrier();
  for (int it = 0; tile < ntiles; tile += gridDim.x, ++it) {
    f16* panel = panels + (it & 1) * (MA_PIX * MA_F * C);
    const int next = tile + (int)gridDim.x;
    f16* other = panels + ((it + 1) & 1) * (MA_PIX * MA_F * C);
    MA_STAMP(2);
    if constexpr (CROSS) {
      if (next < ntiles) fetch_rows(next, other);
      __builtin_amdgcn_sched_barrier(0);
    }

    f16x4 qh[MA_PIX][DT];
    project(panel, rs_w, w_wave, std::true_type{}, zero_init, no_hook);
#pragma unroll
    for (int pix = 0; pix < MA_PIX; ++pix)
#pragma unroll
      for (int t = 0; t < DT; ++t) qh[pix][t] = to_half(CROSS ? acc[pix][t] * scale_log2 : acc[pix][t]);
    MA_STAMP(3);
    if constexpr (CROSS && OUTP) lds_barrier();

    if constexpr (CROSS) {
      const int ctx = tile / p.tiles_per_ctx;
      const f16* cf = reinterpret_cast<const f16*>(p.ctx_frag) + ((int64_t)ctx * H + wave) * (2 * MA_KT * DT * 256) + lane * 4;
      f16x4 kf[MA_KT][DT], vf[DT][MA_KT];
#pragma unroll
      for (int kt = 0; kt < MA_KT; ++kt)
#pragma unroll
        for (int t = 0; t < DT; ++t) {
          kf[kt][t] = *reinterpret_cast<const f16x4*>(cf + (kt * DT + t) * 256);
          vf[t][kt] = *reinterpret_cast<const f16x4*>(cf + (MA_KT * DT + t * MA_KT + kt) * 256);
        }
      const bool has_ip = p.ip_len > 0;
      f16x4 kfi[DT], vfi[DT];
      if (has_ip) {
        const f16* ci = reinterpret_cast<const f16*>(p.ip_frag) + ((int64_t)ctx * H + wave) * (2 * MA_KT * DT * 256) + lane * 4;
#pragma unroll
        for (int t = 0; t < DT; ++t) {
          kfi[t] = *reinterpret_cast<const f16x4*>(ci + t * 256);
          vfi[t] = *reinterpret_cast<const f16x4*>(ci + (MA_KT * DT + t * MA_KT) * 256);
        }
      }
      MA_STAMP(4);
      MA_STAMP(5);
      f16* __restrict__ O = reinterpret_cast<f16*>(p.out) + (int64_t)tile * (MA_PIX * MA_F) * p.ldo + wave * D;
      const int sln = ma_opaque(lane), sg = sln >> 4, sl15 = sln & 15;
#pragma unroll
      for (int pix = 0; pix < MA_PIX; ++pix) {
        float sv[MA_KT][4];
        float mx = -INFINITY;
#pragma unroll
        for (int kt = 0; kt < MA_KT; ++kt) {
          f32x4 sacc = {0.f, 0.f, 0.f, 0.f};
#pragma unroll
          for (int t = 0; t < DT; ++t) sacc = mfma16x16x16(kf[kt][t], qh[pix][t], sacc);
#pragma unroll
          for (int r = 0; r < 4; ++r) {
            const bool live = (kt < MA_KT - 1 && p.lt > 16 * (MA_KT - 1)) || 16 * kt + 4 * g + r < p.lt;
            sv[kt][r] = live ? sacc[r] : -INFINITY;
            mx = fmaxf(mx, sv[kt][r]);
          }
        }
        mx = lane_xor32_max(lane_xor16_max(mx));
        float ls = 0.f;
#pragma unroll
        for (int kt = 0; kt < MA_KT; ++kt)
#pragma unroll
          for (int r = 0; r < 4; ++r) {
            sv[kt][r] = __builtin_amdgcn_exp2f(sv[kt][r] - mx);
            ls += sv[kt][r];
          }
        ls = lane_xor32_sum(lane_xor16_sum(ls));
        const float inv = 1.0f / ls;
        f16x4 pk[MA_KT];
#pragma unroll
        for (int kt = 0; kt < MA_KT; ++kt) pk[kt] = f16x4{(f16)sv[kt][0], (f16)sv[kt][1], (f16)sv[kt][2], (f16)sv[kt][3]};
        f32x4 ov[DT];
#pragma unroll
        for (int t = 0; t < DT; ++t) {
          f32x4 o = {0.f, 0.f, 0.f, 0.f};
#pragma unroll
          for (int kt = 0; kt < MA_KT; ++kt) o = mfma16x16x16(vf[t][kt], pk[kt], o);
          ov[t] = o * inv;
        }
        if (has_ip) {
          f32x4 sacc = {0.f, 0.f, 0.f, 0.f};
#pragma unroll
          for (int t = 0; t < DT; ++t) sacc = mfma16x16x16(kfi[t], qh[pix][t], sacc);
          float si[4];
          float mi = -INFINITY;
#pragma unroll
          for (int r = 0; r < 4; ++r) {
            si[r] = (4 * g + r < p.ip_len) ? sacc[r] : -INFINITY;
            mi = fmaxf(mi, si[r]);
          }
          mi = lane_xor32_max(lane_xor16_max(mi));
          float li = 0.f;
#pragma unroll
          for (int r = 0; r < 4; ++r) {
            si[r] = __builtin_amdgcn_exp2f(si[r] - mi);
            li += si[r];
          }
          li = lane_xor32_sum(lane_xor16_sum(li));
          const float wi = p.ip_scale / li;
          const f16x4 pi = {(f16)si[0], (f16)si[1], (f16)si[2], (f16)si[3]};
#pragma unroll
          for (int t = 0; t < DT; ++t) ov[t] += mfma16x16x16(vfi[t], pi, f32x4{0.f, 0.f, 0.f, 0.f}) * wi;
        }
        u32x2 oh[DT];
#pragma unroll
        for (int t = 0; t < DT; ++t) oh[t] = __builtin_bit_cast(u32x2, to_half(ov[t]));
        if constexpr (OUTP)
          stash_o(panel, pix, oh);
        else
          store_tiles(O + (int64_t)(16 * pix + sl15) * p.ldo, sg, oh);
      }
      MA_STAMP(6);
      if (next < ntiles) normalise_rows(other);
      if constexpr (OUTP) {
        lds_barrier();
        out_project(panel, tile);
      }
    } else {
    constexpr int NB = F == 32 ? 2 : 1;
    f16x4 ph[MA_PIX][NB];
    project(panel, rs_w, w_wave + DP * C * 2, std::true_type{}, zero_init, no_hook);
#pragma unroll
    for (int px = 0; px < MA_PIX; px += NB) {
#pragma unroll
      for (int jq = 0; jq < NB; ++jq) {
        float sv[NB][4];
        float mx = -INFINITY;
#pragma unroll
        for (int ik = 0; ik < NB; ++ik) {
          f32x4 sacc = {0.f, 0.f, 0.f, 0.f};
#pragma unroll
          for (int t = 0; t < DT; ++t) sacc = mfma16x16x16(to_half(acc[px + ik][t]), qh[px + jq][t], sacc);
#pragma unroll
          for (int r = 0; r < 4; ++r) {
            sv[ik][r] = sacc[r] * scale_log2;
            if (F == 8 && (g >> 1) != (l15 >> 3)) sv[ik][r] = -INFINITY;
            mx = fmaxf(mx, sv[ik][r]);
          }
        }
        mx = lane_xor32_max(lane_xor16_max(mx));
        float ls = 0.f;
#pragma unroll
        for (int ik = 0; ik < NB; ++ik)
#pragma unroll
          for (int r = 0; r < 4; ++r) {
            sv[ik][r] = __builtin_amdgcn_exp2f(sv[ik][r] - mx);
            ls += sv[ik][r];
          }
        ls = lane_xor32_sum(lane_xor16_sum(ls));
        const float inv = 1.0f / ls;
#pragma unroll
        for (int ik = 0; ik < NB; ++ik)
          ph[px + ik][jq] = f16x4{(f16)(sv[ik][0] * inv), (f16)(sv[ik][1] * inv), (f16)(sv[ik][2] * inv), (f16)(sv[ik][3] * inv)};
      }
    }
    MA_STAMP(4);

    if (next < ntiles) fetch_rows(next, other);
    __builtin_amdgcn_sched_barrier(0);

    project(panel, rs_w, w_wave + 2 * (DP * C * 2), std::false_type{}, zero_init, no_hook);
    MA_STAMP(5);
    if constexpr (OUTP) lds_barrier();
    f16* __restrict__ O = reinterpret_cast<f16*>(p.out) + (int64_t)tile * (MA_PIX * MA_F) * p.ldo + wave * D;
    const int sln = ma_opaque(lane), sg = sln >> 4, sl15 = sln & 15;
#pragma unroll
    for (int px = 0; px < MA_PIX; px += NB)
#pragma unroll
      for (int jq = 0; jq < NB; ++jq) {
        u32x2 oh[DT];
#pragma unroll
        for (int t = 0; t < DT; ++t) {
          f32x4 o = {0.f, 0.f, 0.f, 0.f};
#pragma unroll
          for (int ik = 0; ik < NB; ++ik) o = mfma16x16x16(to_half(acc[px + ik][t]), ph[px + ik][jq], o);
          oh[t] = __builtin_bit_cast(u32x2, to_half(o));
        }
        if constexpr (OUTP)
          stash_o(panel, px + jq, oh);
        else
          store_tiles(O + (int64_t)(16 * (px + jq) + sl15) * p.ldo, sg, oh);
      }
    MA_STAMP(6);
    if (next < ntiles) normalise_rows(other);
    if constexpr (OUTP) {
      lds_barrier();
      out_project(panel, tile);
    }
    }
    MA_STAMP(7);
#ifdef I2V_MA_STAMPS
    if (stamps != nullptr && lane == 0 && it < 4) {
      long long* st = stamps + (((int64_t)blockIdx.x * 4 + it) * H + wave) * 8;
#pragma unroll
      for (int k = 0; k < 8; ++k) st[k] = stamp[k];
    }
#endif
    lds_barrier();
  }
#undef MA_STAMP
}

template <int C, int D, int H, bool CROSS, int F = 16, bool OUTP = false>
int ma_cus() {
  return i2v_big_lds_kernel_cus(reinterpret_cast<const void*>(motion_attn_kernel<C, D, H, CROSS, F, OUTP>), 2 * (size_t)MA_PIX * MA_F * C * sizeof(f16));
}

template <int C, int D, int H, bool CROSS, int F = 16, bool OUTP = false>
int launch_ma(const ma_args& p, int64_t rows, float scale, hipStream_t s, const char* what) {
  const size_t lds = 2 * (size_t)MA_PIX * MA_F * C * sizeof(f16);
  const int cus = ma_cus<C, D, H, CROSS, F, OUTP>();
  if (cus <= 0) I2V_FAIL(I2V_ERR_UNSUPPORTED, "%s: %zu bytes of LDS refused by this device", what, lds);
  const int ntiles = (int)(rows / (MA_PIX * MA_F));
  const int grid = i2v_persistent_grid(ntiles, cus);
  long long* stamps = nullptr;
#ifdef I2V_MA_STAMPS
  stamps = getenv("I2V_MA_STAMP_PTR") ? reinterpret_cast<long long*>(strtoull(getenv("I2V_MA_STAMP_PTR"), nullptr, 0)) : nullptr;
#endif
  hipLaunchKernelGGL((motion_attn_kernel<C, D, H, CROSS, F, OUTP>), dim3((unsigned)grid), dim3(64 * H), lds, s, p, scale * 1.4426950408889634f,
                     ntiles, stamps);
  return i2v_check_launch(what);
}

}

extern "C" int32_t i2v_motion_attn_supported(int64_t rows, int32_t channels, int32_t heads, int32_t head_dim, int32_t frames) {
  return rows > 0 && rows % (MA_PIX * MA_F) == 0 && rows / (MA_PIX * MA_F) < (1 << 24) && channels == 320 && heads == 8 &&
         head_dim == 40 &&
         ((frames == 16 && ma_cus<320, 40, 8, false, 16>() > 0) || (frames == 8 && ma_cus<320, 40, 8, false, 8>() > 0) ||
          (frames == 32 && ma_cus<320, 40, 8, false, 32>() > 0));
}

extern "C" int32_t i2v_motion_attn_pack_rows(int32_t heads, int32_t head_dim) { return heads * 3 * ((head_dim + 15) / 16) * 16; }

extern "C" int i2v_motion_attn_f16(const i2v_motion_attn_params* pp, i2v_stream_t stream) {
  I2V_CHECK_ARG(pp != nullptr, "i2v_motion_attn_f16: null params");
  const i2v_motion_attn_params& p = *pp;
  I2V_CHECK_ARG(p.x && p.gamma && p.shift && p.w_qkv && p.out, "i2v_motion_attn_f16: null pointer");
  I2V_CHECK_ARG(i2v_motion_attn_supported(p.rows, p.channels, p.heads, p.head_dim, p.frames),
                "i2v_motion_attn_f16: rows %lld channels %d heads %d head_dim %d frames %d is not a fused shape "
                "(i2v_motion_attn_supported)", (long long)p.rows, p.channels, p.heads, p.head_dim, p.frames);
  I2V_CHECK_ARG(p.ldx >= p.channels && p.ldx % 8 == 0 && p.ldo >= p.channels && p.ldo % 8 == 0 && p.ld_shift >= p.channels &&
                p.ld_shift % 4 == 0, "i2v_motion_attn_f16: row strides");
  I2V_CHECK_ARG(i2v_al16(p.x) && i2v_al16(p.gamma) && i2v_al16(p.shift) && i2v_al16(p.w_qkv) && i2v_al16(p.out),
                "i2v_motion_attn_f16: pointers must be 16-byte aligned");
  ma_args a = {};
  a.x = p.x; a.ldx = p.ldx; a.gamma = p.gamma; a.shift = p.shift; a.ld_shift = p.ld_shift; a.w = p.w_qkv; a.out = p.out;
  a.ldo = p.ldo; a.eps = p.eps;
  I2V_CHECK_ARG(p.w_o == nullptr || p.ldx < (1 << 23), "i2v_motion_attn_f16: ldx (%lld) must be below 2^23 with the out-projection", (long long)p.ldx);
  I2V_CHECK_ARG((p.w_o == nullptr) == (p.b_o == nullptr) && i2v_al16(p.w_o) && i2v_al16(p.b_o),
                "i2v_motion_attn_f16: w_o and b_o come together, 16-byte aligned");
  a.w_o = p.w_o; a.b_o = p.b_o;
  hipStream_t s = reinterpret_cast<hipStream_t>(stream);
  if (p.w_o != nullptr) {
    if (p.frames == 8) return launch_ma<320, 40, 8, false, 8, true>(a, p.rows, p.scale, s, "i2v_motion_attn_f16");
    if (p.frames == 32) return launch_ma<320, 40, 8, false, 32, true>(a, p.rows, p.scale, s, "i2v_motion_attn_f16");
    return launch_ma<320, 40, 8, false, 16, true>(a, p.rows, p.scale, s, "i2v_motion_attn_f16");
  }
  if (p.frames == 8) return launch_ma<320, 40, 8, false, 8>(a, p.rows, p.scale, s, "i2v_motion_attn_f16");
  if (p.frames == 32) return launch_ma<320, 40, 8, false, 32>(a, p.rows, p.scale, s, "i2v_motion_attn_f16");
  return launch_ma<320, 40, 8, false, 16>(a, p.rows, p.scale, s, "i2v_motion_attn_f16");
}

extern "C" int32_t i2v_cross_attn_fused_supported(int64_t rows, int32_t channels, int32_t heads, int32_t head_dim, int32_t ctx_len,
                                                  int64_t rows_per_ctx) {
  return rows > 0 && rows % (MA_PIX * MA_F) == 0 && rows / (MA_PIX * MA_F) < (1 << 24) && channels == 320 && heads == 8 &&
         head_dim == 40 && ctx_len >= 1 && ctx_len <= 16 * MA_KT && rows_per_ctx > 0 && rows_per_ctx % (MA_PIX * MA_F) == 0 &&
         rows % rows_per_ctx == 0 && ma_cus<320, 40, 8, true>() > 0;
}

extern "C" int32_t i2v_cross_attn_fused_pack_rows(int32_t heads, int32_t head_dim) { return heads * ((head_dim + 15) / 16) * 16; }

extern "C" int64_t i2v_cross_attn_fused_ctx_elems(int32_t n_ctx, int32_t heads, int32_t head_dim) {
  return (int64_t)n_ctx * heads * 2 * MA_KT * ((head_dim + 15) / 16) * 256;
}

extern "C" int i2v_cross_attn_fused_f16(const i2v_cross_attn_fused_params* pp, i2v_stream_t stream) {
  I2V_CHECK_ARG(pp != nullptr, "i2v_cross_attn_fused_f16: null params");
  const i2v_cross_attn_fused_params& p = *pp;
  I2V_CHECK_ARG(p.x && p.gamma && p.beta && p.w_q && p.ctx_frag && p.out, "i2v_cross_attn_fused_f16: null pointer");
  I2V_CHECK_ARG(i2v_cross_attn_fused_supported(p.rows, p.channels, p.heads, p.head_dim, p.ctx_len, p.rows_per_ctx),
                "i2v_cross_attn_fused_f16: rows %lld channels %d heads %d head_dim %d ctx_len %d rows_per_ctx %lld is not a fused shape "
                "(i2v_cross_attn_fused_supported)", (long long)p.rows, p.channels, p.heads, p.head_dim, p.ctx_len,
                (long long)p.rows_per_ctx);
  I2V_CHECK_ARG(p.ldx >= p.channels && p.ldx % 8 == 0 && p.ldo >= p.channels && p.ldo % 8 == 0, "i2v_cross_attn_fused_f16: row strides");
  I2V_CHECK_ARG(i2v_al16(p.x) && i2v_al16(p.gamma) && i2v_al16(p.beta) && i2v_al16(p.w_q) && i2v_al16(p.out) && i2v_al16(p.ctx_frag) && i2v_al16(p.ip_frag),
                "i2v_cross_attn_fused_f16: pointers must be 16-byte aligned");
  I2V_CHECK_ARG(p.ip_frag == nullptr || (p.ip_len >= 1 && p.ip_len <= 16), "i2v_cross_attn_fused_f16: ip_len (%d) must be in [1, 16]",
                p.ip_len);
  ma_args a = {};
  a.x = p.x; a.ldx = p.ldx; a.gamma = p.gamma; a.shift = p.beta; a.ld_shift = 0; a.w = p.w_q; a.out = p.out; a.ldo = p.ldo;
  a.eps = p.eps;
  a.ctx_frag = p.ctx_frag; a.lt = p.ctx_len;
  a.ip_frag = p.ip_frag; a.ip_len = p.ip_frag ? p.ip_len : 0; a.ip_scale = p.ip_scale;
  a.tiles_per_ctx = (int32_t)(p.rows_per_ctx / (MA_PIX * MA_F));
  I2V_CHECK_ARG(p.w_o == nullptr || p.ldx < (1 << 23), "i2v_cross_attn_fused_f16: ldx (%lld) must be below 2^23 with the out-projection", (long long)p.ldx);
  I2V_CHECK_ARG((p.w_o == nullptr) == (p.b_o == nullptr) && i2v_al16(p.w_o) && i2v_al16(p.b_o),
                "i2v_cross_attn_fused_f16: w_o and b_o come together, 16-byte aligned");
  a.w_o = p.w_o; a.b_o = p.b_o;
  if (p.w_o != nullptr)
    return launch_ma<320, 40, 8, true, 16, true>(a, p.rows, p.scale, reinterpret_cast<hipStream_t>(stream), "i2v_cross_attn_fused_f16");
  return launch_ma<320, 40, 8, true>(a, p.rows, p.scale, reinterpret_cast<hipStream_t>(stream), "i2v_cross_attn_fused_f16");
}
```

### i2v-adapter-unofficial_amd/handle.py

```python
import bisect
import ctypes as C
import struct

import torch

from . import _lib

PLAN_MAGIC, PLAN_VERSION = 0x50563249, 1
ENTRY_IDS = {name: i for i, name in enumerate((
    "i2v_gemm_f16", "i2v_attention_f16", "i2v_temporal_attention_f16", "i2v_motion_attn_f16", "i2v_cross_attn_fused_f16", "i2v_ln_qkv_f16",
    "i2v_ff_fused_f16", "i2v_groupnorm_f16", "i2v_layernorm_f16", "i2v_groupnorm_fold_f16", "i2v_nchw_to_tokens", "i2v_tokens_to_nchw",
    "i2v_timestep_embedding", "i2v_silu_f16", "i2v_repeat_rows_f16", "i2v_copy3d_f16", "i2v_select_row_f16",
    "i2v_pack_ctx_fragments_f16", "i2v_ddim_prep", "i2v_ddim_cfg_step", "i2v_dpm_cfg_step"))}
LATER_ENTRY_IDS = {name: len(ENTRY_IDS) + i for i, name in enumerate((
    "i2v_freeu_f16",
    "i2v_lcm_cfg_step",
    "i2v_freenoise_gather_f16", "i2v_freenoise_blend_f16"))}
ENTRY_NAMES = {i: n for n, i in {**ENTRY_IDS, "i2v_freeu_f16": LATER_ENTRY_IDS["i2v_freeu_f16"]}.items()}


def entry_id(name):
    return ENTRY_IDS.get(name, LATER_ENTRY_IDS.get(name))


def entry_name(i):
    return next((n for n, j in {**ENTRY_IDS, **LATER_ENTRY_IDS}.items() if j == i), None)


IO_SAMPLE, IO_TIMESTEPS, IO_CONTEXT, IO_IMAGE_EMBEDS, IO_OUT = range(5)
RELOC_ARENA, RELOC_WEIGHT, RELOC_IO = range(3)
_INT_TYPES = (C.c_int32, C.c_int64, C.c_int)


def _pad8(n):
    return (n + 7) & ~7


class _RecordingLib:

    def __init__(self, real):
        self._real = real
        self.ops = []

    def __getattr__(self, name):
        fn = getattr(self._real, name)
        if not name.startswith("i2v_") or name not in _lib.SIGNATURES:
            return fn
        res, argtypes = _lib.SIGNATURES[name]
        launches = bool(argtypes) and argtypes[-1] is C.c_void_p and res is C.c_int and not name.startswith("i2v_unet_")
        if not launches:
            return fn
        if entry_id(name) is None:
            def refuse(*a, _n=name):
                raise _lib.HipLibraryError(f"{_n} is not an entry point a launch plan can carry (handle.entry_id / csrc/handle.hip)")
            return refuse

        def call(*args, _n=name, _fn=fn, _at=argtypes):
            self._log(_n, args, _at)
            return _fn(*args)
        return call

    def _log(self, name, args, argtypes):
        if len(args) != len(argtypes):
            raise TypeError(f"{name}: {len(args)} arguments for {len(argtypes)} parameters")
        sbytes, slots, ptrs = b"", [], []
        for arg, at in zip(args[:-1], argtypes[:-1]):
            if isinstance(at, type) and issubclass(at, C._Pointer) and issubclass(at._type_, C.Structure):
                st = arg._obj
                if sbytes or slots:
                    raise TypeError(f"{name}: the parameter struct must come first")
                sbytes = bytes(st)
                for fname, ftype in st._fields_:
                    if ftype is C.c_void_p:
                        v = getattr(st, fname)
                        if v:
                            ptrs.append((getattr(type(st), fname).offset, int(v), f"{name}.{fname}"))
            elif at is C.c_void_p:
                v = arg.value if isinstance(arg, C.c_void_p) else arg
                v = int(v) if v else 0
                if v:
                    ptrs.append((_pad8(len(sbytes)) + 8 * len(slots), v, f"{name} argument {len(slots)}"))
                slots.append(struct.pack("<Q", v))
            elif at in _INT_TYPES:
                slots.append(struct.pack("<q", int(arg)))
            elif at is C.c_float:
                slots.append(struct.pack("<d", float(arg)))
            else:
                raise TypeError(f"{name}: a launch plan carries pointers, integers and floats, not {at}")
        self.ops.append((entry_id(name), sbytes, slots, ptrs))


def persistent_tensors(unet):
    out = {}

    def add(name, v):
        if torch.is_tensor(v):
            if v.is_cuda and v.numel():
                out[name] = v
        elif isinstance(v, (tuple, list)):
            for i, e in enumerate(v):
                add(f"{name}#{i}", e)

    for mname, m in unet.named_modules():
        packed = getattr(m, "_packed", None)
        if isinstance(packed, dict):
            for k, v in dict.items(packed):
                add(f"{mname}#{k}", v)
        for (site, frames), tab in getattr(m, "_ma_tables", {}).items():
            add(f"{mname}#ma_table{site}_{frames}", tab)
    from .free_noise import persistent_tables
    for k, v in persistent_tables(next(unet.parameters()).device).items():
        add(k, v)
    tp = getattr(unet, "_temb_packed", None)
    if tp is not None:
        add("#temb_proj", tp[:2])
    for k, v in unet.state_dict().items():
        add(k, v)
    return out


def _storage_range(t):
    st = t.untyped_storage()
    return st.data_ptr(), st.data_ptr() + st.nbytes()


def pack_plan(keys, ops_bin, relocs, payload, problem, arena_bytes, io_mask):
    key_tab = bytearray()
    for k in keys:
        kb = k.encode() if isinstance(k, str) else bytes(k)
        key_tab += struct.pack("<I", len(kb)) + kb + b"\0" * (-len(kb) % 4)
    key_tab += b"\0" * (-len(key_tab) % 8)
    hdr_size = struct.calcsize("<6I6iQ2I6Q")
    keys_off = hdr_size
    ops_off = keys_off + len(key_tab)
    relocs_off = ops_off + 24 * len(ops_bin)
    payload_off = relocs_off + 24 * len(relocs)
    total = payload_off + len(payload)
    hdr = struct.pack("<6I6iQ2I6Q", PLAN_MAGIC, PLAN_VERSION, _lib.ABI_VERSION, len(ops_bin), len(keys), len(relocs),
                      *[int(v) for v in problem], arena_bytes, io_mask, 0,
                      keys_off, ops_off, relocs_off, payload_off, len(payload), total)
    blob = bytes(hdr + key_tab + b"".join(ops_bin) + b"".join(relocs) + bytes(payload))
    assert len(blob) == total
    return blob


def pack_op(entry, struct_bytes, slots, relocations, payload, relocs):
    blockb = bytearray(struct_bytes) + bytearray(_pad8(len(struct_bytes)) - len(struct_bytes))
    for v in slots:
        blockb += v
    begin = len(relocs)
    for off, kind, index, addend in relocations:
        if off + 8 <= len(blockb):
            blockb[off: off + 8] = b"\0" * 8
        relocs.append(struct.pack("<IIIIQ", off, kind, index, 0, addend))
    rec = struct.pack("<IIIIII", entry, len(payload), len(blockb), begin, len(relocs) - begin, len(struct_bytes))
    payload += blockb
    return rec


def record_plan(run, *, unet, io, problem, late_io=None, extra_persistent=None, restore=None):
    dev = next(iter(io.values())).device
    for t in io.values():
        if not t.is_cuda or not t.is_contiguous():
            raise ValueError("record_plan: the arguments must be contiguous device tensors")
    with torch.no_grad():
        if restore is not None:
            restore()
        run()
        torch.cuda.synchronize(dev)
        if restore is not None:
# ... 387 lines not shown
```

### i2v-adapter-unofficial_amd/kernels.py

```python
import ctypes as C
import functools
import os
from typing import Optional

import torch

from . import _lib
from ._lib import (I2V_A_CONV3X3, I2V_A_PLAIN, I2V_EPI_GEGLU, I2V_EPI_GELU, I2V_EPI_NONE, I2V_STORE_ROWMAJOR,
                   I2V_STORE_ROWPERM, I2V_STORE_VT, I2V_STORE_VT_T, AttnBwdParams, AttnParams, GemmParams, GnParams,
                   HipLibraryError, LnParams, TAttnParams)

f16 = torch.float16


def _stream():
    return C.c_void_p(torch.cuda.current_stream().cuda_stream)


def _req(t: torch.Tensor, name: str, dtype=f16):
    if not isinstance(t, torch.Tensor):
        raise TypeError(f"{name} must be a tensor")
    if not t.is_cuda:
        raise HipLibraryError(f"{name} is on {t.device}: the I2V-Adapter HIP path has no CPU fallback "
                              "(move tensors to a ROCm device)")
# ... 551 lines not shown
        raise ValueError(f"cross_attn_fused: w_q is {tuple(w_q.shape)} (pack_cross_q)")
    if out is None:
        out = torch.empty((rows, c), dtype=f16, device=x.device)
    out, ldo = _mat(out, "out")
    p = _lib.CrossAttnFusedParams()
    p.x, p.ldx = _p(x), ldx
    p.gamma, p.beta, p.w_q = _p(gamma32), _p(beta32), _p(w_q)
    p.ctx_frag = _p(ctx_frag)
    p.out, p.ldo = _p(out), ldo
    p.rows, p.rows_per_ctx = rows, rows_per_ctx
    p.channels, p.heads, p.head_dim, p.ctx_len = c, heads, head_dim, ctx_len
    p.eps, p.scale = float(eps), float(head_dim) ** -0.5 if scale is None else float(scale)
    if ip_frag is not None:
        _req(ip_frag, "ip_frag")
        if not ip_frag.is_contiguous() or ip_frag.numel() != ctx_frag.numel():
            raise ValueError(f"cross_attn_fused: ip_frag is {tuple(ip_frag.shape)} (pack_ctx_fragments of the image tokens)")
        p.ip_frag, p.ip_len, p.ip_scale = _p(ip_frag), int(ip_len), float(ip_scale)
    if out_proj is not None:
        p.w_o, p.b_o = _attn_out_operands(out_proj, c, heads, head_dim, "cross_attn_fused")
    _lib.check(lib.i2v_cross_attn_fused_f16(C.byref(p), _stream()), "i2v_cross_attn_fused_f16")
    return out


def ln_qkv_supported(rows, channels, n_qk, rows_per_image):
    return bool(_lib.load().i2v_ln_qkv_supported(rows, channels, n_qk, rows_per_image))


def pack_ln_qkv(w_qk, w_v):
    w = torch.cat([w_qk.detach().to(f16), w_v.detach().to(f16)], dim=0)
    n, c = w.shape
    if n % 160 or c % 32:
        raise ValueError(f"pack_ln_qkv: {n} rows x {c} columns is not whole waves of 160 rows / K steps of 32")
    return w.view(n // 16, 16, c // 32, 4, 8).permute(0, 2, 3, 1, 4).contiguous().view(n, c)


def ln_qkv(x, gamma32, beta32, w_packed, *, n_qk, rows_per_image, eps, qk=None, vt=None, images=None, x_image_stride=0):
    lib = _lib.load()
    x, ldx = _mat(x, "x")
    rows, c = x.shape
    if images is not None:
        if x_image_stride % ldx or (images - 1) * (x_image_stride // ldx) + rows_per_image > rows:
            raise ValueError(f"ln_qkv: {images} images of {rows_per_image} rows at stride {x_image_stride} do not fit x {tuple(x.shape)}")
        rows = images * rows_per_image
    _req(w_packed, "w")
    for name, t in (("gamma32", gamma32), ("beta32", beta32)):
        _req(t, name, dtype=torch.float32)
    if tuple(gamma32.shape) != (c,) or tuple(beta32.shape) != (c,) or tuple(w_packed.shape) != (n_qk + c, c) or \
            not w_packed.is_contiguous():
        raise ValueError(f"ln_qkv: gamma {tuple(gamma32.shape)}, beta {tuple(beta32.shape)}, w {tuple(w_packed.shape)} for C {c}, "
                         f"n_qk {n_qk} (pack_ln_qkv)")
    if rows % rows_per_image:
        raise ValueError(f"ln_qkv: {rows} rows are not whole images of {rows_per_image}")
    n_img, ld = rows // rows_per_image, pad8(rows_per_image)
    if qk is None:
        qk = torch.empty((rows, n_qk), dtype=f16, device=x.device)
    if vt is None:
        vt = torch.empty((n_img, c, ld), dtype=f16, device=x.device)
    qk, ld_qk = _mat(qk, "qk")
    _req(vt, "vt")
    if tuple(qk.shape) != (rows, n_qk) or tuple(vt.shape) != (n_img, c, ld) or not vt.is_contiguous():
        raise ValueError(f"ln_qkv: qk {tuple(qk.shape)}, vt {tuple(vt.shape)}")
    p = _lib.LnQkvParams()
    p.x, p.ldx = _p(x), ldx
    p.gamma, p.beta, p.w = _p(gamma32), _p(beta32), _p(w_packed)
    p.qk, p.ld_qk = _p(qk), ld_qk
    p.vt, p.vt_batch_stride, p.vt_row_stride = _p(vt), c * ld, ld
    p.rows, p.rows_per_image, p.channels, p.n_qk, p.eps = rows, rows_per_image, c, n_qk, float(eps)
    p.x_image_stride = int(x_image_stride) if images is not None else 0
    _lib.check(lib.i2v_ln_qkv_f16(C.byref(p), _stream()), "i2v_ln_qkv_f16")
    return qk, vt


def ff_fused_supported(rows, channels, inner):
    return bool(_lib.load().i2v_ff_fused_supported(rows, channels, inner))


def pack_ff_fused(w1, b1, w2, b2):
    inner, c = w2.shape[1], w2.shape[0]
    nch, heads, dn = inner // 128, 8, c // 8
    dt = (dn + 15) // 16
    dev = w1.device
    m = torch.arange(16, device=dev)
    idx = ((m & 1) * inner + (m >> 1))[None, None, None, :] + (128 * torch.arange(nch, device=dev))[:, None, None, None] + \
        (16 * torch.arange(8, device=dev))[None, :, None, None] + (8 * torch.arange(2, device=dev))[None, None, :, None]
    t1 = w1.detach().to(f16)[idx.reshape(-1)].view(nch, 8, 2, 16, c // 32, 4, 8)
    w1f = t1.permute(0, 1, 2, 4, 5, 3, 6).contiguous().view(-1, 8)
    b1f = b1.detach().float()[idx.reshape(-1)].view(nch, 8, 2, 16).contiguous()
    w2p = torch.zeros((heads, 16 * dt, inner), dtype=f16, device=dev)
    w2p[:, :dn] = w2.detach().to(f16).view(heads, dn, inner)
    t2 = w2p.view(heads, dt, 16, nch, 4, 4, 8)
    w2f = t2.permute(0, 3, 4, 1, 5, 2, 6).contiguous().view(-1, 8)
    return w1f, b1f, w2f, b2.detach().float().contiguous()


def ff_fused_tail_supported(rows, channels, inner, perm_frames=0, perm_hw=0):
    return bool(_lib.load().i2v_ff_fused_tail_supported(rows, channels, inner, perm_frames, perm_hw))


def pack_ff_tail(w3, b3):
    return pack_cross_q(w3, 8), b3.detach().float().contiguous()


def ff_fused(x, gamma32, beta32, packed, *, eps, out=None, tail=None, precise=False):
    lib = _lib.load()
    x, ldx = _mat(x, "x")
    rows, c = x.shape
    w1f, b1f, w2f, b2f = packed
    inner = b1f.numel() // 2
    for name, t, dt_ in (("gamma32", gamma32, torch.float32), ("beta32", beta32, torch.float32), ("w1", w1f, f16),
                         ("b1", b1f, torch.float32), ("w2", w2f, f16), ("b2", b2f, torch.float32)):
        _req(t, name, dtype=dt_)
    if tuple(gamma32.shape) != (c,) or tuple(beta32.shape) != (c,) or b2f.numel() != c or w1f.numel() != 2 * inner * c or \
            w2f.numel() != 8 * ((c // 8 + 15) // 16 * 16) * inner:
        raise ValueError(f"ff_fused: operand sizes do not match C {c}, inner {inner} (pack_ff_fused)")
    if out is None:
        out = torch.empty((rows, c), dtype=f16, device=x.device)
    out, ldo = _mat(out, "out")
    if tuple(out.shape) != (rows, c):
        raise ValueError(f"ff_fused: out is {tuple(out.shape)}")
    p = _lib.FfFusedParams()
    p.x, p.ldx = _p(x), ldx
    p.gamma, p.beta = _p(gamma32), _p(beta32)
    p.w1, p.b1, p.w2, p.b2 = _p(w1f), _p(b1f), _p(w2f), _p(b2f)
    p.out, p.ldo = _p(out), ldo
    p.rows, p.channels, p.inner, p.eps = rows, c, inner, float(eps)
    keep = None
    if tail is not None:
        (w3f, b3f), res2, perm_frames, perm_hw = tail
        _req(w3f, "w3")
        _req(b3f, "b3", dtype=torch.float32)
        res2, ld2 = _mat(res2, "res2")
        if tuple(w3f.shape) != (8 * ((c // 8 + 15) // 16 * 16), c) or not w3f.is_contiguous() or b3f.numel() != c or \
                tuple(res2.shape) != (rows, c):
            raise ValueError(f"ff_fused: tail operands w3 {tuple(w3f.shape)}, b3 {tuple(b3f.shape)}, res2 {tuple(res2.shape)} "
                             f"do not match rows {rows}, C {c} (pack_ff_tail)")
        if perm_frames and out.data_ptr() == x.data_ptr():
            raise ValueError("ff_fused: out must not alias x when the tail permutes the rows")
        p.w3, p.b3, p.res2, p.ld_res2 = _p(w3f), _p(b3f), _p(res2), ld2
        p.perm_frames, p.perm_hw = int(perm_frames), int(perm_hw)
        if precise and lo_of(res2) is not None:
            def set_lo(rl, cl):
                p.res2_lo, p.out_lo = _p(rl), _p(cl)
            keep = _attach_lo(set_lo, res2, out)
    _lib.check(lib.i2v_ff_fused_f16(C.byref(p), _stream()), "i2v_ff_fused_f16")
    del keep
    return out


def motion_attn_tables(gamma, beta, pe, frames):
    return (gamma.detach().float().contiguous(),
            (beta.detach().float()[None, :] + pe.detach().float()[:frames]).contiguous())


def motion_attn(x, gamma32, shift32, w_qkv, *, heads, head_dim, frames, eps, scale=None, out=None, out_proj=None):
    lib = _lib.load()
    x, ldx = _mat(x, "x")
    rows, c = x.shape
    _req(w_qkv, "w_qkv")
    for name, t in (("gamma32", gamma32), ("shift32", shift32)):
        _req(t, name, dtype=torch.float32)
    if c != heads * head_dim or tuple(gamma32.shape) != (c,) or tuple(shift32.shape) != (frames, c) or not shift32.is_contiguous():
        raise ValueError(f"motion_attn: C {c} vs heads {heads} x head_dim {head_dim}, gamma {tuple(gamma32.shape)}, "
                         f"shift {tuple(shift32.shape)} (expected [{frames}, {c}])")
    if tuple(w_qkv.shape) != (lib.i2v_motion_attn_pack_rows(heads, head_dim), c) or not w_qkv.is_contiguous():
        raise ValueError(f"motion_attn: w_qkv is {tuple(w_qkv.shape)} (pack_motion_qkv)")
    if out is None:
        out = torch.empty((rows, c), dtype=f16, device=x.device)
    out, ldo = _mat(out, "out")
    if tuple(out.shape) != (rows, c):
        raise ValueError(f"motion_attn: out is {tuple(out.shape)}")
    p = _lib.MotionAttnParams()
    p.x, p.ldx = _p(x), ldx
    p.gamma = _p(gamma32)
    p.shift, p.ld_shift = _p(shift32), c
    p.w_qkv = _p(w_qkv)
    p.out, p.ldo = _p(out), ldo
    p.rows, p.channels, p.heads, p.head_dim, p.frames = rows, c, heads, head_dim, frames
    p.eps, p.scale = float(eps), float(head_dim) ** -0.5 if scale is None else float(scale)
    if out_proj is not None:
        p.w_o, p.b_o = _attn_out_operands(out_proj, c, heads, head_dim, "motion_attn")
    _lib.check(lib.i2v_motion_attn_f16(C.byref(p), _stream()), "i2v_motion_attn_f16")
    return out


def groupnorm(x, gamma, beta, groups, eps, *, x2=None, silu=False, frames_per_stat=1, out_perm=False, frames=0, stats=None):
    lib = _lib.load()
    _req(x, "x")
    if x.dim() != 4 or not x.is_contiguous():
        raise ValueError(f"x must be contiguous [N, H, W, C], got {tuple(x.shape)}")
    n, h, w, c1 = x.shape
    c2 = 0
    if x2 is not None:
        _req(x2, "x2")
        if x2.dim() != 4 or not x2.is_contiguous() or x2.shape[:3] != x.shape[:3]:
            raise ValueError("x2 must be contiguous [N, H, W, C2] with the same N, H, W as x")
        c2 = x2.shape[3]
    Cc = c1 + c2
    _req(gamma, "gamma")
    _req(beta, "beta")
    if gamma.numel() != Cc or beta.numel() != Cc:
        raise ValueError(f"gamma / beta must have {Cc} elements")
    ws = torch.empty((lib.i2v_groupnorm_workspace_bytes(n, h * w, Cc) + 3) // 4, dtype=torch.float32, device=x.device)
    y = torch.empty((n * h * w, Cc) if out_perm else (n, h, w, Cc), dtype=f16, device=x.device)
    p = GnParams()
    p.x, p.c1, p.x2, p.c2 = _p(x), c1, _p(x2), c2
    p.gamma, p.beta, p.y = _p(gamma.contiguous()), _p(beta.contiguous()), _p(y)
    p.n_img, p.hw, p.groups, p.frames_per_stat = n, h * w, groups, frames_per_stat
    p.eps, p.silu = eps, 1 if silu else 0
    p.out_perm, p.frames = (1 if out_perm else 0), frames
    p.workspace = _p(ws)
    if stats is not None:
        part, rows = stats
        _req(part, "stats", dtype=torch.float32)
        if x2 is not None or frames_per_stat != 1 or out_perm or tuple(part.shape) != (n, (h * w) // rows, groups, 2) or \
                not part.is_contiguous():
            raise ValueError(f"groupnorm: stats {tuple(part.shape)} / rows {rows} do not describe x {tuple(x.shape)} in {groups} groups")
        p.gpartial_in, p.gpartial_rows = _p(part), int(rows)
    _lib.check(lib.i2v_groupnorm_f16(C.byref(p), _stream()), "i2v_groupnorm_f16")
    return y


def groupnorm_fold(x, gamma, beta, groups, eps, w, bias, *, x2=None, frames_per_stat=1):
    lib = _lib.load()
    _req(x, "x")
    if x.dim() != 4 or not x.is_contiguous():
        raise ValueError(f"x must be contiguous [N, H, W, C], got {tuple(x.shape)}")
    n, h, wd, c1 = x.shape
    c2 = 0
    if x2 is not None:
        _req(x2, "x2")
        if x2.dim() != 4 or not x2.is_contiguous() or x2.shape[:3] != x.shape[:3]:
            raise ValueError("x2 must be contiguous [N, H, W, C2] with the same N, H, W as x")
        c2 = x2.shape[3]
    Cc = c1 + c2
    _req(gamma, "gamma")
    _req(beta, "beta")
    w2, ldw = _mat(w, "w")
    if gamma.numel() != Cc or beta.numel() != Cc or w2.shape[1] != Cc:
        raise ValueError(f"gamma / beta / w columns must have {Cc} elements")
    n_out = w2.shape[0]
    if bias is not None:
        _req(bias, "bias")
        if bias.numel() != n_out or not bias.is_contiguous():
            raise ValueError("bias must be a contiguous vector of n_out elements")
    if frames_per_stat <= 0 or n % frames_per_stat != 0:
        raise ValueError(f"batch {n} is not a multiple of frames_per_stat {frames_per_stat}")
    S = n // frames_per_stat
    ws = torch.empty((lib.i2v_groupnorm_workspace_bytes(n, h * wd, Cc) + 3) // 4, dtype=torch.float32, device=x.device)
    w_s = torch.empty((S, n_out, Cc), dtype=f16, device=x.device)
    b_s = torch.empty((S, n_out), dtype=f16, device=x.device)
    p = GnParams()
    p.x, p.c1, p.x2, p.c2 = _p(x), c1, _p(x2), c2
    p.gamma, p.beta = _p(gamma.contiguous()), _p(beta.contiguous())
    p.n_img, p.hw, p.groups, p.frames_per_stat = n, h * wd, groups, frames_per_stat
    p.eps = eps
    p.workspace = _p(ws)
    _lib.check(lib.i2v_groupnorm_fold_f16(C.byref(p), _p(w2), ldw, _p(bias), n_out, _p(w_s), _p(b_s), _stream()),
               "i2v_groupnorm_fold_f16")
    return w_s, b_s


def layernorm(x, gamma, beta, eps, *, pe=None, pe_period=0):
    lib = _lib.load()
    batched = None
    if x.dim() == 3:
        _req(x, "x")
        if x.stride(2) != 1 or x.stride(1) % 8 != 0 or x.stride(0) % 8 != 0 or x.stride(0) <= 0:
            raise ValueError("batched layernorm input needs unit last stride and row / batch strides that are multiples of 8")
        batched = (x.shape[1], x.stride(0))
        ldx = x.stride(1)
        rows, Cc = x.shape[0] * x.shape[1], x.shape[2]
    else:
        x, ldx = _mat(x, "x")
        rows, Cc = x.shape
    _req(gamma, "gamma")
    _req(beta, "beta")
    y = torch.empty((rows, Cc), dtype=f16, device=x.device)
    p = LnParams()
    p.x, p.ldx = _p(x), ldx
    p.gamma, p.beta = _p(gamma), _p(beta)
    if pe is not None:
        pe, ldpe = _mat(pe, "pe")
        if pe.shape[1] != Cc or pe.shape[0] < pe_period or pe_period <= 0:
            raise ValueError("pe must be [>= pe_period, C]")
        p.pe, p.ld_pe, p.pe_period = _p(pe), ldpe, pe_period
    p.y, p.ldy = _p(y), Cc
    p.rows, p.C, p.eps = rows, Cc, eps
    if batched is not None:
        p.x_rows_per_batch, p.x_batch_stride = batched
    _lib.check(lib.i2v_layernorm_f16(C.byref(p), _stream()), "i2v_layernorm_f16")
    return y


def softmax_rows(x, scale=1.0, out=None):
    lib = _lib.load()
    x, ldx = _mat(x, "x")
    if out is None:
        out = torch.empty((x.shape[0], pad8(x.shape[1])), dtype=f16, device=x.device)[:, : x.shape[1]]
    out, ldy = _mat(out, "out")
    if out.shape != x.shape:
        raise ValueError("softmax_rows: out must have x's shape")
    _lib.check(lib.i2v_softmax_rows_f16(_p(x), ldx, _p(out), ldy, x.shape[0], x.shape[1], float(scale), _stream()),
               "i2v_softmax_rows_f16")
    return out


def nchw_to_tokens(src, c_pad=None):
    lib = _lib.load()
    _req(src, "src", dtype=None)
    if src.dtype not in (torch.float32, f16) or src.dim() != 4:
        raise TypeError("src must be a 4-D fp32 / fp16 tensor")
    src = src.contiguous()
    n, c, h, w = src.shape
    c_pad = c if c_pad is None else c_pad
    dst = torch.empty((n, h, w, c_pad), dtype=f16, device=src.device)
    _lib.check(lib.i2v_nchw_to_tokens(_p(src), 1 if src.dtype == torch.float32 else 0, _p(dst), n, c, h * w, c_pad,
                                      _stream()), "i2v_nchw_to_tokens")
    return dst


def tokens_to_nchw(src, c=None, dtype=f16):
    lib = _lib.load()
    _req(src, "src", dtype=None)
    if src.dtype not in (torch.float32, f16):
        raise TypeError("src must be fp16 or fp32")
    if src.dim() != 4 or not src.is_contiguous():
        raise ValueError("src must be contiguous [N, H, W, C]")
    n, h, w, ld = src.shape
    c = ld if c is None else c
    if dtype not in (torch.float32, f16):
        raise TypeError("dtype must be fp32 or fp16")
    dst = torch.empty((n, c, h, w), dtype=dtype, device=src.device)
    _lib.check(lib.i2v_tokens_to_nchw(_p(src), 1 if src.dtype == torch.float32 else 0, ld, _p(dst),
                                      1 if dtype == torch.float32 else 0, n, c, h * w, _stream()), "i2v_tokens_to_nchw")
# ... 1036 lines not shown
```

### include/i2v_hip.h

```cpp
#ifndef I2V_HIP_H
#define I2V_HIP_H

#include <stdint.h>

#ifdef __cplusplus
extern "C" {
#endif

#define I2V_ABI_VERSION 27

#define I2V_OK 0
#define I2V_ERR_INVALID_ARG (-1)
#define I2V_ERR_UNSUPPORTED (-2)
#define I2V_ERR_LAUNCH (-3)

typedef void* i2v_stream_t;

int i2v_abi_version(void);
const char* i2v_last_error(void);

enum {
  I2V_EPI_NONE = 0,
  I2V_EPI_GELU = 1,
  I2V_EPI_GEGLU = 2
};

enum {
  I2V_STORE_ROWMAJOR = 0,
  I2V_STORE_ROWPERM = 1,
  I2V_STORE_VT = 2,
  I2V_STORE_VT_T = 3
};

enum {
  I2V_A_PLAIN = 0,
  I2V_A_CONV3X3 = 1
};

typedef struct i2v_gemm_params {
  const void* a;
  int64_t lda;
  const void* a2;
  int64_t lda2;
  int32_t k_split;
  int32_t a_mode;
  const void* w;
  int64_t ldw;
  const void* bias;
  const void* residual;
  int64_t ldr;
  const void* rowvec;
  int64_t ld_rowvec;
  int32_t rows_per_vec;
  int32_t rowvec_period;
  const void* ln_wsum;
  float ln_eps;
  void* c;
  int64_t ldc;
  int32_t M, N, K;
  int32_t epilogue;
  int32_t store_mode;
  int32_t frames, hw;
  int32_t vt_len, vt_ld;
  float out_scale;
  int32_t n_img, in_h, in_w, cin, out_h, out_w, stride, upsample, asym_pad;
  int32_t conv_kblock;
  int64_t w_batch_stride;
  int32_t rows_per_w;
  int32_t a_perm_frames, a_perm_hw;
  void* workspace;
  int64_t workspace_bytes;
  int32_t c_is_f32;
  void* gn_partial;
  int32_t gn_groups;
  const void* residual_lo;
  void* c_lo;
} i2v_gemm_params;

int i2v_gemm_f16(const i2v_gemm_params* p, i2v_stream_t stream);
int i2v_gemm_ln_supported(const i2v_gemm_params* p);
int i2v_gemm_batch_supported(const i2v_gemm_params* p);
int i2v_gemm_upconv_fold_supported(const i2v_gemm_params* p);
int64_t i2v_gemm_workspace_bytes(const i2v_gemm_params* p);
int32_t i2v_gemm_gn_partial_rows(const i2v_gemm_params* p);

enum {
  I2V_ROUTE_GENERIC = 0,
  I2V_ROUTE_CONV_THIN = 1,
  I2V_ROUTE_BIG_TILE = 2,
  I2V_ROUTE_BIG_DEEP = 3,
  I2V_ROUTE_BIG_SPLITK = 4
};
enum { I2V_EXTRA_NONE = 0, I2V_EXTRA_LNF = 1, I2V_EXTRA_HILO = 2, I2V_EXTRA_GNS = 4, I2V_EXTRA_UPF = 8 };

struct i2v_gemm_route {
  int32_t family;
  int32_t a_mode;
  int32_t rows, cols;
  int32_t stages;
  int32_t splits, kps;
  int32_t extra;
  int32_t persistent;
  int32_t generic_tile;
  int32_t vec4;
  int32_t epilogue;
  int32_t store_mode;
};

int i2v_gemm_route(const i2v_gemm_params* p, struct i2v_gemm_route* route);
int i2v_gemm_last_route(struct i2v_gemm_route* route);
int i2v_gemm_kernel_exists(const struct i2v_gemm_route* route);

typedef struct i2v_attn_params {
  const void* q;  int64_t q_row_stride, q_batch_stride;
  const void* k;  int64_t k_row_stride, k_batch_stride;
  const void* vt; int64_t vt_row_stride, vt_batch_stride;
  void* o;        int64_t o_row_stride, o_batch_stride;
  int32_t batch_q, kv_group, heads, head_dim, lq, lk;
  float scale;
  int32_t accumulate;
  float acc_scale;
  float* lse;
} i2v_attn_params;

int i2v_attention_f16(const i2v_attn_params* p, i2v_stream_t stream);

typedef struct i2v_tattn_params {
  const void* q; int64_t q_row_stride;
  const void* k; int64_t k_row_stride;
  const void* vt; int32_t vt_ld;
  void* o; int64_t o_row_stride;
  int32_t n_pixels, frames, heads, head_dim;
  float scale;
} i2v_tattn_params;

int i2v_temporal_attention_f16(const i2v_tattn_params* p, i2v_stream_t stream);

enum { I2V_TATTN_LDS_FORM = 0, I2V_TATTN_REG_FORM = 1 };

struct i2v_tattn_route {
  int32_t form;
  int32_t dqk, dpv;
  int32_t pf;
  int32_t nqt;
  int32_t blocks;
};

int i2v_temporal_attention_route(const i2v_tattn_params* p, struct i2v_tattn_route* route);
int i2v_temporal_attention_last_route(struct i2v_tattn_route* route);
int i2v_tattn_kernel_exists(const struct i2v_tattn_route* route);

typedef struct i2v_motion_attn_params {
  const void* x; int64_t ldx;
  const void* gamma;
  const void* shift; int64_t ld_shift;
  const void* w_qkv;
  void* out; int64_t ldo;
  int64_t rows;
  int32_t channels, heads, head_dim, frames;
  float eps, scale;
  const void* w_o; const void* b_o;
} i2v_motion_attn_params;

int32_t i2v_motion_attn_supported(int64_t rows, int32_t channels, int32_t heads, int32_t head_dim, int32_t frames);
int32_t i2v_motion_attn_pack_rows(int32_t heads, int32_t head_dim);
int i2v_motion_attn_f16(const i2v_motion_attn_params* p, i2v_stream_t stream);

typedef struct i2v_cross_attn_fused_params {
  const void* x; int64_t ldx;
  const void* gamma; const void* beta;
  const void* w_q;
  const void* ctx_frag;
  void* out; int64_t ldo;
  int64_t rows, rows_per_ctx;
  int32_t channels, heads, head_dim, ctx_len;
  float eps, scale;
  const void* ip_frag; int32_t ip_len; float ip_scale;
  const void* w_o; const void* b_o;
} i2v_cross_attn_fused_params;

int32_t i2v_cross_attn_fused_supported(int64_t rows, int32_t channels, int32_t heads, int32_t head_dim, int32_t ctx_len,
                                       int64_t rows_per_ctx);
int32_t i2v_cross_attn_fused_pack_rows(int32_t heads, int32_t head_dim);
int64_t i2v_cross_attn_fused_ctx_elems(int32_t n_ctx, int32_t heads, int32_t head_dim);
int i2v_cross_attn_fused_f16(const i2v_cross_attn_fused_params* p, i2v_stream_t stream);

typedef struct i2v_ln_qkv_params {
  const void* x; int64_t ldx;
  const void* gamma; const void* beta;
  const void* w;
  void* qk; int64_t ld_qk;
  void* vt; int64_t vt_batch_stride, vt_row_stride;
  int64_t rows, rows_per_image;
  int32_t channels, n_qk;
  float eps;
  int64_t x_image_stride;
} i2v_ln_qkv_params;

int32_t i2v_ln_qkv_supported(int64_t rows, int32_t channels, int32_t n_qk, int64_t rows_per_image);
int i2v_ln_qkv_f16(const i2v_ln_qkv_params* p, i2v_stream_t stream);

typedef struct i2v_ff_fused_params {
  const void* x; int64_t ldx;
  const void* gamma; const void* beta;
  const void* w1; const void* b1;
  const void* w2; const void* b2;
  void* out; int64_t ldo;
  int64_t rows;
  int32_t channels, inner;
  float eps;
  const void* w3; const void* b3;
  const void* res2; int64_t ld_res2;
  int32_t perm_frames, perm_hw;
  const void* res2_lo;
  void* out_lo;
} i2v_ff_fused_params;

int32_t i2v_ff_fused_supported(int64_t rows, int32_t channels, int32_t inner);
int32_t i2v_ff_fused_tail_supported(int64_t rows, int32_t channels, int32_t inner, int32_t perm_frames, int32_t perm_hw);
int i2v_ff_fused_f16(const i2v_ff_fused_params* p, i2v_stream_t stream);

typedef struct i2v_gn_params {
  const void* x;  int32_t c1;
  const void* x2; int32_t c2;
  const void* gamma; const void* beta;
  void* y;
  int32_t n_img, hw, groups, frames_per_stat;
  float eps;
  int32_t silu;
  int32_t out_perm; int32_t frames;
  void* workspace;
  const void* gpartial_in; int32_t gpartial_rows;
} i2v_gn_params;

int64_t i2v_groupnorm_workspace_bytes(int32_t n_img, int32_t hw, int32_t channels);
int i2v_groupnorm_f16(const i2v_gn_params* p, i2v_stream_t stream);
int i2v_groupnorm_fold_f16(const i2v_gn_params* p, const void* w, int64_t ldw, const void* bias, int32_t n_out,
                           void* w_out, void* bias_out, i2v_stream_t stream);

typedef struct i2v_ln_params {
  const void* x; int64_t ldx;
  const void* gamma; const void* beta;
  const void* pe; int64_t ld_pe; int32_t pe_period;
  void* y; int64_t ldy;
  int32_t rows, C;
  float eps;
  int32_t x_rows_per_batch; int64_t x_batch_stride;
} i2v_ln_params;

int i2v_layernorm_f16(const i2v_ln_params* p, i2v_stream_t stream);

int i2v_softmax_rows_f16(const void* x, int64_t ldx, void* y, int64_t ldy, int32_t rows, int32_t cols, float scale,
                         i2v_stream_t stream);

int i2v_nchw_to_tokens(const void* src, int32_t src_is_f32, void* dst, int32_t n, int32_t c, int32_t hw,
                       int32_t c_pad, i2v_stream_t stream);
int i2v_tokens_to_nchw(const void* src, int32_t src_is_f32, int64_t ld, void* dst, int32_t dst_is_f32, int32_t n,
                       int32_t c, int32_t hw, i2v_stream_t stream);
int i2v_timestep_embedding(const float* t, const int32_t* t_index, int32_t t_rows, void* out, int32_t n,
                           int32_t dim, i2v_stream_t stream);
int i2v_select_row_f16(const void* table, int64_t ld, int32_t rows, const int32_t* row_index, void* out, int32_t cols,
                       i2v_stream_t stream);
int i2v_silu_f16(const void* x, void* y, int64_t n, i2v_stream_t stream);
int i2v_repeat_rows_f16(const void* x, void* y, int64_t rows_in, int64_t cols, int32_t repeat,
                        i2v_stream_t stream);
int i2v_copy3d_f16(const void* src, int64_t src_batch_stride, int64_t ld_src, void* dst, int64_t dst_batch_stride,
                   int64_t ld_dst, int64_t batches, int64_t rows, int64_t cols, i2v_stream_t stream);

int64_t i2v_pack_ctx_fragments_elems(int32_t n_ctx, int32_t heads, int32_t head_dim);
int i2v_pack_ctx_fragments_f16(const void* k, int64_t ldk, const void* vt, int64_t vt_row_stride, int64_t vt_batch_stride, void* out,
                               int32_t n_ctx, int32_t heads, int32_t head_dim, int32_t ctx_len, i2v_stream_t stream);

int i2v_ddim_prep(float* latents, const float* cond, void* model_in, int32_t b, int32_t f, int32_t c,
                  int32_t hw, int32_t c_pad, int32_t cfg_copies, i2v_stream_t stream);
int i2v_ddim_cfg_step(float* latents, const void* noise_pred, int32_t np_is_f32, int64_t ld_np, const float* coef, int32_t n_steps,
                      int32_t* step_index, float guidance_scale, int32_t b, int32_t f, int32_t c, int32_t hw,
                      int32_t cfg_copies, i2v_stream_t stream);

int i2v_dpm_cfg_step(float* latents, float* x0_prev, const void* noise_pred, int32_t np_is_f32, int64_t ld_np, const float* coef,
                     int32_t n_steps, int32_t* step_index, float guidance_scale, int32_t b, int32_t f, int32_t c, int32_t hw,
                     int32_t cfg_copies, i2v_stream_t stream);

int i2v_lcm_cfg_step(float* latents, const float* noise, int32_t n_noise, const void* noise_pred, int32_t np_is_f32, int64_t ld_np,
                     const float* coef, int32_t n_steps, int32_t* step_index, float guidance_scale, int32_t b, int32_t f, int32_t c,
                     int32_t hw, int32_t cfg_copies, i2v_stream_t stream);

int i2v_freeu_f16(const void* hidden, const void* hidden_lo, void* hidden_out, void* hidden_out_lo, const void* skip, void* skip_out,
                  int32_t n, int32_t h, int32_t w, int32_t c1, int32_t c2, float b, float s, i2v_stream_t stream);

int i2v_vae_tile_blend(const void* tile, const void* up, const void* left, const void* upleft, int32_t src_is_f32, int32_t n, int32_t th,
                       int32_t tw, int64_t ld, int32_t c, int32_t up_h, int32_t left_w, int32_t blend_extent, int32_t limit, void* out,
                       int32_t out_h, int32_t out_w, int32_t oy, int32_t ox, i2v_stream_t stream);

#define I2V_LORA_MAX_ADAPTERS 8
#define I2V_LORA_MAX_RANK 256
typedef struct i2v_lora_adapter {
  const void* down;
  const void* up;
  int32_t rank;
  float scale;
} i2v_lora_adapter;
int i2v_lora_merge(void* dst, const void* base, int32_t is_f32, int32_t out, int32_t in, const i2v_lora_adapter* adapters,
                   int32_t n_adapters, i2v_stream_t stream);

int64_t i2v_freeinit_workspace_bytes(int32_t b, int32_t f, int32_t c, int32_t h, int32_t w);
int i2v_freeinit_mix(const float* latents, const float* init_noise, const float* z_rand, const float* lpf, float* out, void* workspace,
                     int64_t workspace_bytes, int32_t b, int32_t f, int32_t c, int32_t h, int32_t w, float sqrt_alpha,
                     float sqrt_one_minus_alpha, i2v_stream_t stream);

int i2v_freenoise_gather_f16(const void* src, int64_t ld_src, void* dst, int64_t ld_dst, const int32_t* starts, int64_t n_pixels,
                             int32_t frames, int32_t windows, int32_t length, int32_t c, i2v_stream_t stream);
int i2v_freenoise_blend_f16(const void* src, int64_t ld_src, void* dst, int64_t ld_dst, const int32_t* idx, const float* coef,
                            int64_t n_pixels, int32_t frames, int32_t windows, int32_t length, int32_t pairs, int32_t c,
                            i2v_stream_t stream);

int i2v_clip_embed_f16(const void* tok, const void* pos, const int32_t* ids, const int32_t* ids_host, void* out, int32_t batch, int32_t len,
                       int32_t vocab, int32_t max_positions, int32_t hidden, i2v_stream_t stream);
int i2v_clip_attention_f16(const void* qkv, int64_t ld_qkv, int32_t q_off, int32_t k_off, int32_t v_off, void* out, int64_t ld_out,
                           int32_t batch, int32_t len, int32_t heads, int32_t head_dim, float scale, i2v_stream_t stream);
int i2v_quick_gelu_f16(const void* x, void* y, int64_t n, i2v_stream_t stream);
// ... 177 lines not shown
```

Baseline: 21.20.

## Add wide fused motion-attention kernel for 640-channel, 80-dim head blocks

Extends the fused LayerNorm+QKV+temporal-attention+out-projection motion kernel to the 640-channel, head_dim 80 case. It does this by making pixels per tile a template parameter, adding a five-tile store pattern, and loading gamma/shift tables late to limit register pressure. Motion blocks at that width previously fell back to the unfused path, and now run as one persistent kernel to cut intermediate memory traffic and launches. The risks are higher register and LDS pressure at C=640, and the path is only taken when free-noise is off.

```diff
diff --git a/i2v-adapter-unofficial_amd/_lib.py b/i2v-adapter-unofficial_amd/_lib.py
--- a/i2v-adapter-unofficial_amd/_lib.py
+++ b/i2v-adapter-unofficial_amd/_lib.py
@@ -3,7 +3,7 @@
 
 _HERE = os.path.dirname(os.path.abspath(__file__))
 LIB_PATH = os.environ.get("I2V_LIB_PATH") or os.path.join(_HERE, "libi2v_hip.so")
-ABI_VERSION = 27
+ABI_VERSION = 28
 
 I2V_EPI_NONE, I2V_EPI_GELU, I2V_EPI_GEGLU = 0, 1, 2
 I2V_STORE_ROWMAJOR, I2V_STORE_ROWPERM, I2V_STORE_VT, I2V_STORE_VT_T = 0, 1, 2, 3
@@ -267,6 +267,8 @@
     "i2v_motion_attn_supported": (C.c_int32, [C.c_int64, C.c_int32, C.c_int32, C.c_int32, C.c_int32]),
     "i2v_motion_attn_pack_rows": (C.c_int32, [C.c_int32, C.c_int32]),
     "i2v_motion_attn_f16": (C.c_int, [C.POINTER(MotionAttnParams), _P]),
+    "i2v_motion_attn_wide_supported": (C.c_int32, [C.c_int64, C.c_int32, C.c_int32, C.c_int32, C.c_int32]),
+    "i2v_motion_attn_wide_f16": (C.c_int, [C.POINTER(MotionAttnParams), _P]),
     "i2v_cross_attn_fused_supported": (C.c_int32, [C.c_int64, C.c_int32, C.c_int32, C.c_int32, C.c_int32, C.c_int64]),
     "i2v_cross_attn_fused_pack_rows": (C.c_int32, [C.c_int32, C.c_int32]),
     "i2v_cross_attn_fused_ctx_elems": (C.c_int64, [C.c_int32, C.c_int32, C.c_int32]),
diff --git a/i2v-adapter-unofficial_amd/blocks.py b/i2v-adapter-unofficial_amd/blocks.py
--- a/i2v-adapter-unofficial_amd/blocks.py
+++ b/i2v-adapter-unofficial_amd/blocks.py
@@ -611,6 +611,7 @@
 FUSED_FF = os.environ.get("I2V_FF_FUSED", "1") != "0"
 FUSED_FF_TAIL = os.environ.get("I2V_FF_TAIL", "1") != "0"
 FUSED_ATTN_OUT = os.environ.get("I2V_ATTN_OUTP", "1") != "0"
+FUSED_MOTION_ATTN_WIDE = os.environ.get("I2V_MOTION_FUSED_WIDE", "1") != "0"
 
 
 class TemporalTransformerBlock(HipModule):
@@ -703,11 +704,17 @@
         c = self.dim
         overlap = t.shape[0] <= streams.MAX_ROWS
         fused = FUSED_MOTION_ATTN and K.motion_attn_supported(t.shape[0], c, self.heads, self.dim_head, frames)
+        wide = (not fused and FUSED_MOTION_ATTN and FUSED_ATTN_OUT and FUSED_MOTION_ATTN_WIDE and self.free_noise is None and
+                K.motion_attn_wide_supported(t.shape[0], c, self.heads, self.dim_head, frames))
         for i in (1, 2):
-            if fused:
+            if fused or wide:
                 tab = self._ma_tables.get((i, frames))
                 if tab is None:
                     tab = self._ma_tables[(i, frames)] = K.motion_attn_tables(p[f"g{i}"], p[f"b{i}"], p["pe"], frames)
+                if wide:
+                    t = K.motion_attn_wide(t, tab[0], tab[1], p[f"wqkv{i}"], heads=self.heads, head_dim=self.dim_head, frames=frames,
+                                           eps=self.eps, out_proj=p[f"wo_frag{i}"])
+                    continue
                 if FUSED_ATTN_OUT:
                     t = K.motion_attn(t, tab[0], tab[1], p[f"wqkv{i}"], heads=self.heads, head_dim=self.dim_head, frames=frames,
                                       eps=self.eps, out_proj=p[f"wo_frag{i}"])
diff --git a/i2v-adapter-unofficial_amd/csrc/handle.hip b/i2v-adapter-unofficial_amd/csrc/handle.hip
--- a/i2v-adapter-unofficial_amd/csrc/handle.hip
+++ b/i2v-adapter-unofficial_amd/csrc/handle.hip
@@ -30,7 +30,7 @@
   E_GEMM = 0, E_ATTN, E_TATTN, E_MOTION_ATTN, E_CROSS_ATTN_FUSED, E_LN_QKV, E_FF_FUSED, E_GROUPNORM, E_LAYERNORM,
   E_GROUPNORM_FOLD, E_NCHW_TO_TOKENS, E_TOKENS_TO_NCHW, E_TIMESTEP_EMBEDDING, E_SILU, E_REPEAT_ROWS, E_COPY3D, E_SELECT_ROW,
   E_PACK_CTX_FRAGMENTS, E_DDIM_PREP, E_DDIM_CFG_STEP, E_DPM_CFG_STEP, E_FREEU, E_LCM_CFG_STEP, E_FREENOISE_GATHER,
-  E_FREENOISE_BLEND, E_COUNT
+  E_FREENOISE_BLEND, E_MOTION_ATTN_WIDE, E_COUNT
 };
 struct EntryInfo {
   const char* name;
@@ -63,6 +63,7 @@
     {"i2v_lcm_cfg_step", 0, 15},
     {"i2v_freenoise_gather_f16", 0, 10},
     {"i2v_freenoise_blend_f16", 0, 12},
+    {"i2v_motion_attn_wide_f16", sizeof(i2v_motion_attn_params), 0},
 };
 inline uint32_t pad8(uint32_t n) { return (n + 7u) & ~7u; }
 
@@ -410,6 +411,7 @@
         rc = i2v_freenoise_blend_f16(P(0), I(1), P(2), I(3), reinterpret_cast<const int32_t*>(P(4)), reinterpret_cast<const float*>(P(5)), I(6),
                                      (int32_t)I(7), (int32_t)I(8), (int32_t)I(9), (int32_t)I(10), (int32_t)I(11), stream);
         break;
+      case E_MOTION_ATTN_WIDE: rc = i2v_motion_attn_wide_f16(reinterpret_cast<const i2v_motion_attn_params*>(buf), stream); break;
       default: I2V_FAIL(I2V_ERR_UNSUPPORTED, "i2v_unet_forward: launch %u names entry point %u", i, op.entry);
     }
     if (rc != I2V_OK) return rc;
diff --git a/i2v-adapter-unofficial_amd/csrc/motion_attn.hip b/i2v-adapter-unofficial_amd/csrc/motion_attn.hip
--- a/i2v-adapter-unofficial_amd/csrc/motion_attn.hip
+++ b/i2v-adapter-unofficial_amd/csrc/motion_attn.hip
@@ -37,12 +37,14 @@
 
 constexpr int MA_KT = 5;
 
-template <int C, int D, int H, bool CROSS, int F = 16, bool OUTP = false>
+template <int C, int D, int H, bool CROSS, int F = 16, bool OUTP = false, int PIX = MA_PIX>
 __global__ __launch_bounds__(64 * H) void motion_attn_kernel(const ma_args p, const float scale_log2, const int ntiles,
                                                              long long* __restrict__ stamps) {
   constexpr int DT = (D + 15) / 16, DP = 16 * DT, KS = C / 32, NJ = C / 64, PARTS = CROSS ? 1 : 3;
+  constexpr int RW = PIX * MA_F / H, HALVES = RW / 8;
   static_assert(C % 64 == 0 && H == 8, "one wave per head, 8 lanes x C / 64 chunks per row in the LayerNorm pass");
   static_assert(F == 8 || F == 16 || F == 32, "frames per pixel");
+  static_assert(RW % 8 == 0 && PIX % (F == 32 ? 2 : 1) == 0, "whole groups of 8 rows per wave, whole pixels per tile");
   extern __shared__ __attribute__((aligned(16))) f16 panels[];
   const int tid = threadIdx.x, lane = tid & 63, wave = __builtin_amdgcn_readfirstlane(tid >> 6);
   const int g = lane >> 4, l15 = lane & 15, sub = lane & 7;
@@ -57,40 +59,45 @@
 #endif
 
   auto fetch_rows = [&](const int tile, f16* panel) {
-    const f16* base = X + ((int64_t)tile * (MA_PIX * MA_F) + 16 * wave) * p.ldx;
-    const auto rs = __builtin_amdgcn_make_buffer_rsrc(const_cast<f16*>(base), 0, (int)((15 * p.ldx + C) * 2), 0x00020000);
+    const f16* base = X + ((int64_t)tile * (PIX * MA_F) + RW * wave) * p.ldx;
+    const auto rs = __builtin_amdgcn_make_buffer_rsrc(const_cast<f16*>(base), 0, (int)(((RW - 1) * p.ldx + C) * 2), 0x00020000);
     const int ln = ma_opaque(lane);
     const unsigned voff = (unsigned)(((ln >> 3) * p.ldx + (ln & 7) * 8) * 2);
 #pragma unroll
-    for (int half = 0; half < 2; ++half)
+    for (int half = 0; half < HALVES; ++half)
 #pragma unroll
       for (int j = 0; j < NJ; ++j)
-        ma_dma16(rs, panel + 16 * wave * C + (half * NJ + j) * 512, voff, (unsigned)((8 * half * p.ldx + 8 * j * 8) * 2));
+        ma_dma16(rs, panel + RW * wave * C + (half * NJ + j) * 512, voff, (unsigned)((8 * half * p.ldx + 8 * j * 8) * 2));
   };
+  constexpr bool LATE_TABLES = NJ > 5;
   auto normalise_rows = [&](f16* panel) {
-    f16x8 xv[2][NJ];
-#pragma unroll
-    for (int half = 0; half < 2; ++half)
-#pragma unroll
-      for (int j = 0; j < NJ; ++j) xv[half][j] = *reinterpret_cast<const f16x8*>(panel + 16 * wave * C + ((half * NJ + j) * 64 + lane) * 8);
+    f16x8 xv[HALVES][NJ];
+#pragma unroll
+    for (int half = 0; half < HALVES; ++half)
+#pragma unroll
+      for (int j = 0; j < NJ; ++j) xv[half][j] = *reinterpret_cast<const f16x8*>(panel + RW * wave * C + ((half * NJ + j) * 64 + lane) * 8);
     const float* gp = gamma;
     const float* sp = shift;
     asm volatile("" : "+s"(gp), "+s"(sp));
     f32x4 ga[NJ][2];
-#pragma unroll
-    for (int j = 0; j < NJ; ++j) {
-      ga[j][0] = *reinterpret_cast<const f32x4*>(gp + (sub + 8 * j) * 8);
-      ga[j][1] = *reinterpret_cast<const f32x4*>(gp + (sub + 8 * j) * 8 + 4);
-    }
-#pragma unroll
-    for (int half = 0; half < 2; ++half) {
-      const int row = 16 * wave + 8 * half + (lane >> 3);
-      const float* sh = sp + (int64_t)((16 * wave + 8 * half + (lane >> 3)) & (F - 1)) * p.ld_shift;
+    if constexpr (!LATE_TABLES) {
+#pragma unroll
+      for (int j = 0; j < NJ; ++j) {
+        ga[j][0] = *reinterpret_cast<const f32x4*>(gp + (sub + 8 * j) * 8);
+        ga[j][1] = *reinterpret_cast<const f32x4*>(gp + (sub + 8 * j) * 8 + 4);
+      }
+    }
+#pragma unroll
+    for (int half = 0; half < HALVES; ++half) {
+      const int row = RW * wave + 8 * half + (lane >> 3);
+      const float* sh = sp + (int64_t)((RW * wave + 8 * half + (lane >> 3)) & (F - 1)) * p.ld_shift;
       f32x4 sv[NJ][2];
-#pragma unroll
-      for (int j = 0; j < NJ; ++j) {
-        sv[j][0] = *reinterpret_cast<const f32x4*>(sh + (sub + 8 * j) * 8);
-        sv[j][1] = *reinterpret_cast<const f32x4*>(sh + (sub + 8 * j) * 8 + 4);
+      if constexpr (!LATE_TABLES) {
+#pragma unroll
+        for (int j = 0; j < NJ; ++j) {
+          sv[j][0] = *reinterpret_cast<const f32x4*>(sh + (sub + 8 * j) * 8);
+          sv[j][1] = *reinterpret_cast<const f32x4*>(sh + (sub + 8 * j) * 8 + 4);
+        }
       }
       float v[NJ][8];
       float s = 0.f;
@@ -116,6 +123,12 @@
 #pragma unroll
       for (int j = 0; j < NJ; ++j) {
         const int ch = sub + 8 * j;
+        if constexpr (LATE_TABLES) {
+          ga[j][0] = *reinterpret_cast<const f32x4*>(gp + ch * 8);
+          ga[j][1] = *reinterpret_cast<const f32x4*>(gp + ch * 8 + 4);
+          sv[j][0] = *reinterpret_cast<const f32x4*>(sh + ch * 8);
+          sv[j][1] = *reinterpret_cast<const f32x4*>(sh + ch * 8 + 4);
+        }
         f16x8 o;
 #pragma unroll
         for (int e = 0; e < 8; ++e) o[e] = (f16)fmaf(v[j][e] * rstd, ga[j][e >> 2][e & 3], sv[j][e >> 2][e & 3]);
@@ -128,7 +141,7 @@
   const int w_lane = lane * 16, w_wave = wave * (PARTS * DP * C * 2);
   const int sw = l15 & 7;
   const int swz[2] = {(g ^ sw) * 8, ((4 + g) ^ sw) * 8};
-  f32x4 acc[MA_PIX][DT];
+  f32x4 acc[PIX][DT];
   auto zero_init = [](const int, const int) { return f32x4{0.f, 0.f, 0.f, 0.f}; };
   auto no_hook = []() {};
   auto project = [&](const f16* panel, const __amdgpu_buffer_rsrc_t rs, const int wp, auto transposed, auto init, auto hook) {
@@ -139,7 +152,7 @@
     const f16* alane = panel + l15 * C;
     f16x8 wf[MA_PD][DT];
 #pragma unroll
-    for (int pix = 0; pix < MA_PIX; ++pix)
+    for (int pix = 0; pix < PIX; ++pix)
 #pragma unroll
       for (int t = 0; t < DT; ++t) acc[pix][t] = init(pix, t);
 #pragma unroll
@@ -147,16 +160,16 @@
 #pragma unroll
       for (int t = 0; t < DT; ++t) wf[s][t] = ldw(s, t);
     __builtin_amdgcn_sched_barrier(0);
-    constexpr int AD = MA_AD, NI = KS * MA_PIX;
+    constexpr int AD = MA_AD, NI = KS * PIX;
     auto lda = [&](const int i) {
-      return *reinterpret_cast<const f16x8*>(alane + 16 * (i % MA_PIX) * C + 64 * ((i / MA_PIX) >> 1) + swz[(i / MA_PIX) & 1]);
+      return *reinterpret_cast<const f16x8*>(alane + 16 * (i % PIX) * C + 64 * ((i / PIX) >> 1) + swz[(i / PIX) & 1]);
     };
     f16x8 af[AD + 1];
 #pragma unroll
     for (int i = 0; i < AD; ++i) af[i] = lda(i);
 #pragma unroll
     for (int i = 0; i < NI; ++i) {
-      const int s = i / MA_PIX, pix = i % MA_PIX;
+      const int s = i / PIX, pix = i % PIX;
       if (pix == 0 && s + MA_PD - 1 < KS) {
 #pragma unroll
         for (int t = 0; t < DT; ++t) wf[(s + MA_PD - 1) % MA_PD][t] = ldw(s + MA_PD - 1, t);
@@ -174,8 +187,26 @@
     }
   };
   auto to_half = [](const f32x4 a) { return f16x4{(f16)a[0], (f16)a[1], (f16)a[2], (f16)a[3]}; };
-  static_assert(DT == 3 && D == 40, "store pattern of three 16-channel tiles holding 40 channels");
+  static_assert((DT == 3 && D == 40) || (DT == 5 && D == 80), "store pattern of three 16-channel tiles holding 40 channels, or of five full ones");
   auto store_tiles = [&](f16* orow, const int g, const u32x2 (&oh)[DT]) {
+    if constexpr (DT == 5) {
+      u32x2 a = oh[0], b = oh[1], c = oh[2], d = oh[3], e = oh[4], f = oh[4];
+      asm volatile("s_nop 1\n\tv_permlane16_swap_b32 %0, %1\n\tv_permlane16_swap_b32 %2, %3\n\t"
+                   "v_permlane16_swap_b32 %4, %5\n\tv_permlane16_swap_b32 %6, %7\n\t"
+                   "v_permlane16_swap_b32 %8, %9\n\tv_permlane16_swap_b32 %10, %11"
+                   : "+v"(a[0]), "+v"(b[0]), "+v"(a[1]), "+v"(b[1]), "+v"(c[0]), "+v"(d[0]), "+v"(c[1]), "+v"(d[1]), "+v"(e[0]), "+v"(f[0]),
+                     "+v"(e[1]), "+v"(f[1]));
+      const int pair = (g & 1) ? 16 + 4 * (g - 1) : 4 * g;
+#ifdef I2V_MA_NOSTORE
+      if (p.ldo < 0)
+#endif
+      {
+        *reinterpret_cast<u32x4*>(orow + pair) = u32x4{a[0], a[1], b[0], b[1]};
+        *reinterpret_cast<u32x4*>(orow + 32 + pair) = u32x4{c[0], c[1], d[0], d[1]};
+        if ((g & 1) == 0) *reinterpret_cast<u32x4*>(orow + 64 + 4 * g) = u32x4{e[0], e[1], f[0], f[1]};
+      }
+      return;
+    }
     u32x2 a = oh[0], b = oh[1], c2 = oh[2], d2 = oh[2];
     asm volatile("s_nop 1\n\tv_permlane16_swap_b32 %0, %1\n\tv_permlane16_swap_b32 %2, %3\n\t"
                  "v_permlane16_swap_b32 %4, %5\n\tv_permlane16_swap_b32 %6, %7"
@@ -202,18 +233,18 @@
   auto out_project = [&](const f16* pr, const int tile) {
     const auto rs_o = __builtin_amdgcn_make_buffer_rsrc(const_cast<void*>(p.w_o), 0, H * DP * C * 2, 0x00020000);
     const auto rs_b = __builtin_amdgcn_make_buffer_rsrc(const_cast<void*>(p.b_o), 0, C * 4, 0x00020000);
-    const f16* base = X + (int64_t)tile * (MA_PIX * MA_F) * p.ldx;
-    const auto rs_x = __builtin_amdgcn_make_buffer_rsrc(const_cast<f16*>(base), 0, (int)(((MA_PIX * MA_F - 1) * p.ldx + C) * 2), 0x00020000);
+    const f16* base = X + (int64_t)tile * (PIX * MA_F) * p.ldx;
+    const auto rs_x = __builtin_amdgcn_make_buffer_rsrc(const_cast<f16*>(base), 0, (int)(((PIX * MA_F - 1) * p.ldx + C) * 2), 0x00020000);
     const int ln = ma_opaque(lane), sg = ln >> 4, sl15 = ln & 15;
     f32x4 bo[DT];
 #pragma unroll
     for (int t = 0; t < DT; ++t)
       bo[t] = __builtin_bit_cast(f32x4, __builtin_amdgcn_raw_buffer_load_b128(
                                             rs_b, 16 * t + 4 * sg < D ? (unsigned)((wave * D + 16 * t + 4 * sg) * 4) : 0x80000000u, 0, 0));
-    u32x2 res[MA_PIX][DT];
+    u32x2 res[PIX][DT];
     project(pr, rs_o, wave * (DP * C * 2), std::true_type{}, [&](const int, const int t) { return bo[t]; }, [&]() {
 #pragma unroll
-      for (int pix = 0; pix < MA_PIX; ++pix)
+      for (int pix = 0; pix < PIX; ++pix)
 #pragma unroll
         for (int t = 0; t < DT; ++t) {
 #ifdef I2V_MA_NORES
@@ -224,9 +255,9 @@
 #endif
         }
     });
-    f16* __restrict__ O = reinterpret_cast<f16*>(p.out) + (int64_t)tile * (MA_PIX * MA_F) * p.ldo + wave * D;
-#pragma unroll
-    for (int pix = 0; pix < MA_PIX; ++pix) {
+    f16* __restrict__ O = reinterpret_cast<f16*>(p.out) + (int64_t)tile * (PIX * MA_F) * p.ldo + wave * D;
+#pragma unroll
+    for (int pix = 0; pix < PIX; ++pix) {
       u32x2 oh[DT];
 #pragma unroll
       for (int t = 0; t < DT; ++t) {
@@ -247,19 +278,19 @@
   MA_STAMP(1);
   lds_barrier();
   for (int it = 0; tile < ntiles; tile += gridDim.x, ++it) {
-    f16* panel = panels + (it & 1) * (MA_PIX * MA_F * C);
+    f16* panel = panels + (it & 1) * (PIX * MA_F * C);
     const int next = tile + (int)gridDim.x;
-    f16* other = panels + ((it + 1) & 1) * (MA_PIX * MA_F * C);
+    f16* other = panels + ((it + 1) & 1) * (PIX * MA_F * C);
     MA_STAMP(2);
     if constexpr (CROSS) {
       if (next < ntiles) fetch_rows(next, other);
       __builtin_amdgcn_sched_barrier(0);
     }
 
-    f16x4 qh[MA_PIX][DT];
+    f16x4 qh[PIX][DT];
     project(panel, rs_w, w_wave, std::true_type{}, zero_init, no_hook);
 #pragma unroll
-    for (int pix = 0; pix < MA_PIX; ++pix)
+    for (int pix = 0; pix < PIX; ++pix)
 #pragma unroll
       for (int t = 0; t < DT; ++t) qh[pix][t] = to_half(CROSS ? acc[pix][t] * scale_log2 : acc[pix][t]);
     MA_STAMP(3);
@@ -288,10 +319,10 @@
       }
       MA_STAMP(4);
       MA_STAMP(5);
-      f16* __restrict__ O = reinterpret_cast<f16*>(p.out) + (int64_t)tile * (MA_PIX * MA_F) * p.ldo + wave * D;
+      f16* __restrict__ O = reinterpret_cast<f16*>(p.out) + (int64_t)tile * (PIX * MA_F) * p.ldo + wave * D;
       const int sln = ma_opaque(lane), sg = sln >> 4, sl15 = sln & 15;
 #pragma unroll
-      for (int pix = 0; pix < MA_PIX; ++pix) {
+      for (int pix = 0; pix < PIX; ++pix) {
         float sv[MA_KT][4];
         float mx = -INFINITY;
 #pragma unroll
@@ -368,10 +399,10 @@
       }
     } else {
     constexpr int NB = F == 32 ? 2 : 1;
-    f16x4 ph[MA_PIX][NB];
+    f16x4 ph[PIX][NB];
     project(panel, rs_w, w_wave + DP * C * 2, std::true_type{}, zero_init, no_hook);
 #pragma unroll
-    for (int px = 0; px < MA_PIX; px += NB) {
+    for (int px = 0; px < PIX; px += NB) {
 #pragma unroll
       for (int jq = 0; jq < NB; ++jq) {
         float sv[NB][4];
@@ -412,10 +443,10 @@
     project(panel, rs_w, w_wave + 2 * (DP * C * 2), std::false_type{}, zero_init, no_hook);
     MA_STAMP(5);
     if constexpr (OUTP) lds_barrier();
-    f16* __restrict__ O = reinterpret_cast<f16*>(p.out) + (int64_t)tile * (MA_PIX * MA_F) * p.ldo + wave * D;
+    f16* __restrict__ O = reinterpret_cast<f16*>(p.out) + (int64_t)tile * (PIX * MA_F) * p.ldo + wave * D;
     const int sln = ma_opaque(lane), sg = sln >> 4, sl15 = sln & 15;
 #pragma unroll
-    for (int px = 0; px < MA_PIX; px += NB)
+    for (int px = 0; px < PIX; px += NB)
 #pragma unroll
       for (int jq = 0; jq < NB; ++jq) {
         u32x2 oh[DT];
@@ -451,23 +482,23 @@
 #undef MA_STAMP
 }
 
-template <int C, int D, int H, bool CROSS, int F = 16, bool OUTP = false>
+template <int C, int D, int H, bool CROSS, int F = 16, bool OUTP = false, int PIX = MA_PIX>
 int ma_cus() {
-  return i2v_big_lds_kernel_cus(reinterpret_cast<const void*>(motion_attn_kernel<C, D, H, CROSS, F, OUTP>), 2 * (size_t)MA_PIX * MA_F * C * sizeof(f16));
-}
-
-template <int C, int D, int H, bool CROSS, int F = 16, bool OUTP = false>
+  return i2v_big_lds_kernel_cus(reinterpret_cast<const void*>(motion_attn_kernel<C, D, H, CROSS, F, OUTP, PIX>), 2 * (size_t)PIX * MA_F * C * sizeof(f16));
+}
+
+template <int C, int D, int H, bool CROSS, int F = 16, bool OUTP = false, int PIX = MA_PIX>
 int launch_ma(const ma_args& p, int64_t rows, float scale, hipStream_t s, const char* what) {
-  const size_t lds = 2 * (size_t)MA_PIX * MA_F * C * sizeof(f16);
-  const int cus = ma_cus<C, D, H, CROSS, F, OUTP>();
+  const size_t lds = 2 * (size_t)PIX * MA_F * C * sizeof(f16);
+  const int cus = ma_cus<C, D, H, CROSS, F, OUTP, PIX>();
   if (cus <= 0) I2V_FAIL(I2V_ERR_UNSUPPORTED, "%s: %zu bytes of LDS refused by this device", what, lds);
-  const int ntiles = (int)(rows / (MA_PIX * MA_F));
+  const int ntiles = (int)(rows / (PIX * MA_F));
   const int grid = i2v_persistent_grid(ntiles, cus);
   long long* stamps = nullptr;
 #ifdef I2V_MA_STAMPS
   stamps = getenv("I2V_MA_STAMP_PTR") ? reinterpret_cast<long long*>(strtoull(getenv("I2V_MA_STAMP_PTR"), nullptr, 0)) : nullptr;
 #endif
-  hipLaunchKernelGGL((motion_attn_kernel<C, D, H, CROSS, F, OUTP>), dim3((unsigned)grid), dim3(64 * H), lds, s, p, scale * 1.4426950408889634f,
+  hipLaunchKernelGGL((motion_attn_kernel<C, D, H, CROSS, F, OUTP, PIX>), dim3((unsigned)grid), dim3(64 * H), lds, s, p, scale * 1.4426950408889634f,
                      ntiles, stamps);
   return i2v_check_launch(what);
 }
@@ -512,6 +543,33 @@
   return launch_ma<320, 40, 8, false, 16>(a, p.rows, p.scale, s, "i2v_motion_attn_f16");
 }
 
+constexpr int MA_WIDE_PIX = 4;
+
+extern "C" int32_t i2v_motion_attn_wide_supported(int64_t rows, int32_t channels, int32_t heads, int32_t head_dim, int32_t frames) {
+  return rows > 0 && rows % (MA_WIDE_PIX * MA_F) == 0 && rows / (MA_WIDE_PIX * MA_F) < (1 << 24) && channels == 640 && heads == 8 &&
+         head_dim == 80 && frames == 16 && ma_cus<640, 80, 8, false, 16, true, MA_WIDE_PIX>() > 0;
+}
+
+extern "C" int i2v_motion_attn_wide_f16(const i2v_motion_attn_params* pp, i2v_stream_t stream) {
+  I2V_CHECK_ARG(pp != nullptr, "i2v_motion_attn_wide_f16: null params");
+  const i2v_motion_attn_params& p = *pp;
+  I2V_CHECK_ARG(p.x && p.gamma && p.shift && p.w_qkv && p.out, "i2v_motion_attn_wide_f16: null pointer");
+  I2V_CHECK_ARG(p.w_o && p.b_o, "i2v_motion_attn_wide_f16: w_o and b_o are required (this form exists only with the out-projection inside)");
+  I2V_CHECK_ARG(i2v_motion_attn_wide_supported(p.rows, p.channels, p.heads, p.head_dim, p.frames),
+                "i2v_motion_attn_wide_f16: rows %lld channels %d heads %d head_dim %d frames %d is not a fused shape "
+                "(i2v_motion_attn_wide_supported)", (long long)p.rows, p.channels, p.heads, p.head_dim, p.frames);
+  I2V_CHECK_ARG(p.ldx >= p.channels && p.ldx % 8 == 0 && p.ldo >= p.channels && p.ldo % 8 == 0 && p.ld_shift >= p.channels &&
+                p.ld_shift % 4 == 0, "i2v_motion_attn_wide_f16: row strides");
+  I2V_CHECK_ARG(i2v_al16(p.x) && i2v_al16(p.gamma) && i2v_al16(p.shift) && i2v_al16(p.w_qkv) && i2v_al16(p.out) && i2v_al16(p.w_o) &&
+                i2v_al16(p.b_o), "i2v_motion_attn_wide_f16: pointers must be 16-byte aligned");
+  I2V_CHECK_ARG(p.ldx < (1 << 23), "i2v_motion_attn_wide_f16: ldx (%lld) must be below 2^23", (long long)p.ldx);
+  ma_args a = {};
+  a.x = p.x; a.ldx = p.ldx; a.gamma = p.gamma; a.shift = p.shift; a.ld_shift = p.ld_shift; a.w = p.w_qkv; a.out = p.out;
+  a.ldo = p.ldo; a.eps = p.eps; a.w_o = p.w_o; a.b_o = p.b_o;
+  return launch_ma<640, 80, 8, false, 16, true, MA_WIDE_PIX>(a, p.rows, p.scale, reinterpret_cast<hipStream_t>(stream),
+                                                              "i2v_motion_attn_wide_f16");
+}
+
 extern "C" int32_t i2v_cross_attn_fused_supported(int64_t rows, int32_t channels, int32_t heads, int32_t head_dim, int32_t ctx_len,
                                                   int64_t rows_per_ctx) {
   return rows > 0 && rows % (MA_PIX * MA_F) == 0 && rows / (MA_PIX * MA_F) < (1 << 24) && channels == 320 && heads == 8 &&
diff --git a/i2v-adapter-unofficial_amd/handle.py b/i2v-adapter-unofficial_amd/handle.py
--- a/i2v-adapter-unofficial_amd/handle.py
+++ b/i2v-adapter-unofficial_amd/handle.py
@@ -15,7 +15,8 @@
 LATER_ENTRY_IDS = {name: len(ENTRY_IDS) + i for i, name in enumerate((
     "i2v_freeu_f16",
     "i2v_lcm_cfg_step",
-    "i2v_freenoise_gather_f16", "i2v_freenoise_blend_f16"))}
+    "i2v_freenoise_gather_f16", "i2v_freenoise_blend_f16",
+    "i2v_motion_attn_wide_f16"))}
 ENTRY_NAMES = {i: n for n, i in {**ENTRY_IDS, "i2v_freeu_f16": LATER_ENTRY_IDS["i2v_freeu_f16"]}.items()}
 
 
diff --git a/i2v-adapter-unofficial_amd/kernels.py b/i2v-adapter-unofficial_amd/kernels.py
--- a/i2v-adapter-unofficial_amd/kernels.py
+++ b/i2v-adapter-unofficial_amd/kernels.py
@@ -727,7 +727,19 @@
             (beta.detach().float()[None, :] + pe.detach().float()[:frames]).contiguous())
 
 
-def motion_attn(x, gamma32, shift32, w_qkv, *, heads, head_dim, frames, eps, scale=None, out=None, out_proj=None):
+def motion_attn_wide_supported(rows, channels, heads, head_dim, frames):
+    return bool(_lib.load().i2v_motion_attn_wide_supported(rows, channels, heads, head_dim, frames))
+
+
+def motion_attn_wide(x, gamma32, shift32, w_qkv, *, heads, head_dim, frames, eps, out_proj, scale=None, out=None):
+    if out_proj is None:
+        raise ValueError("motion_attn_wide: out_proj is required (pack_attn_out)")
+    return motion_attn(x, gamma32, shift32, w_qkv, heads=heads, head_dim=head_dim, frames=frames, eps=eps, scale=scale, out=out,
+                       out_proj=out_proj, _entry="i2v_motion_attn_wide_f16")
+
+
+def motion_attn(x, gamma32, shift32, w_qkv, *, heads, head_dim, frames, eps, scale=None, out=None, out_proj=None,
+                _entry="i2v_motion_attn_f16"):
     lib = _lib.load()
     x, ldx = _mat(x, "x")
     rows, c = x.shape
@@ -754,7 +766,7 @@
     p.eps, p.scale = float(eps), float(head_dim) ** -0.5 if scale is None else float(scale)
     if out_proj is not None:
         p.w_o, p.b_o = _attn_out_operands(out_proj, c, heads, head_dim, "motion_attn")
-    _lib.check(lib.i2v_motion_attn_f16(C.byref(p), _stream()), "i2v_motion_attn_f16")
+    _lib.check(getattr(lib, _entry)(C.byref(p), _stream()), _entry)
     return out
 
 
diff --git a/include/i2v_hip.h b/include/i2v_hip.h
--- a/include/i2v_hip.h
+++ b/include/i2v_hip.h
@@ -7,7 +7,7 @@
 extern "C" {
 #endif
 
-#define I2V_ABI_VERSION 27
+#define I2V_ABI_VERSION 28
 
 #define I2V_OK 0
 #define I2V_ERR_INVALID_ARG (-1)
@@ -166,6 +166,9 @@
 int32_t i2v_motion_attn_pack_rows(int32_t heads, int32_t head_dim);
 int i2v_motion_attn_f16(const i2v_motion_attn_params* p, i2v_stream_t stream);
 
+int32_t i2v_motion_attn_wide_supported(int64_t rows, int32_t channels, int32_t heads, int32_t head_dim, int32_t frames);
+int i2v_motion_attn_wide_f16(const i2v_motion_attn_params* p, i2v_stream_t stream);
+
 typedef struct i2v_cross_attn_fused_params {
   const void* x; int64_t ldx;
   const void* gamma; const void* beta;
```

Result: faster. 21.43 (median of 6 runs) (+1.1%).
